# Sindhu-Hegde/jegal

Hardware: AMD Instinct MI355X
Metric: clips/sec (T=150 frames, 270x480) embedding extraction (higher is better)
Workload: dtype f16; 1 GPU; BASELINE configs[1]: synthetic batch=32 gesture-only (GestSync conv + JEGAL gesture encoder), uint8 150x270x480x3 clips resident in HBM, seeded synthetic weights; clips_per_gpu=32, frames=150, precision_mode=5, chunk=32, conv1_zero_tile_skip=True, dual_stream=True, parallelism=clip-sharded x1, no data-path collective

## Files before the change

### include/jegal_hip.h

```cpp
#ifndef JEGAL_HIP_H
#define JEGAL_HIP_H

#include <stdint.h>

#ifdef __cplusplus
extern "C" {
#endif

typedef struct jg_handle jg_handle;

enum { JG_OK = 0, JG_ERR_ARG = -1, JG_ERR_HIP = -2, JG_ERR_STATE = -3, JG_ERR_WEIGHT = -4 };

enum { JG_F32 = 0, JG_F16 = 1, JG_I64 = 2, JG_U8 = 3 };

enum {
    JG_PREC_FP16 = 0,
    JG_PREC_FP16_W2 = 1,
    JG_PREC_FP16_W2_ALL = 2,
    JG_PREC_FP16_BC = 3,
    JG_PREC_BF16 = 4,
    JG_PREC_FP16_RC = 5,
    JG_PREC_FP32 = 6
};

int jg_create(int device, jg_handle** out);
int jg_destroy(jg_handle* h);
const char* jg_last_error(jg_handle* h);
int jg_set_stream(jg_handle* h, void* hip_stream);
int jg_set_precision(jg_handle* h, int mode);
int jg_set_chunk(jg_handle* h, int clips_per_chunk);
int jg_set_option(jg_handle* h, const char* name, int value);
int jg_sync(jg_handle* h);

int jg_load_tensor(jg_handle* h, const char* name, const void* data_host, const int64_t* shape_host, int ndim, int dtype);
int jg_finalize_weights(jg_handle* h, int which);
int jg_clear_staged_tensors(jg_handle* h);

int jg_calibrate_gesture(jg_handle* h, const void* frames, int frames_dtype, int B, int T);

int jg_xlmr_encode(jg_handle* h, const int32_t* input_ids, const int32_t* attention_mask, int B, int L, float* out);
int jg_calibrate_xlmr(jg_handle* h, const int32_t* input_ids, const int32_t* attention_mask, int B, int L);

int jg_gestsync_clip(jg_handle* h, const void* frames, int frames_dtype, int B, int T, float* out_feats);
int jg_gestsync_clip_ragged(jg_handle* h, const void* frames, int frames_dtype, int B, int T, const int32_t* valid_frames_host, float* out_feats);
int jg_debug_conv1_pool(jg_handle* h, const void* frames_u8, int B, int T, int pad, void* out_f16);
typedef struct jg_gemm_check {
    const void* A; int64_t lda;
    const void* Wh; const void* Wl; int64_t ldw;
    int M, N, K;
    const float* scale; const float* bias;
    const float* bias_clip; int rpc, nclips;
    const float* res; int64_t ldr; int res_mod;
    int relu;
    float* out32; void* out16; int64_t ldc;
    const float* ln_w; const float* ln_b; const void* res16;
    int ln_mode; const float* ln_stats; const void* xres_hi; const void* xres_lo; void* out_lo; float* stat_out;
} jg_gemm_check;
int jg_debug_gemm_check(jg_handle* h, const jg_gemm_check* c);
typedef struct jg_conv_shape { int H, W, C, KH, KW, PH, PW, tap_table, rowmap, const_in; } jg_conv_shape;
int jg_debug_gemm_plan(const jg_gemm_check* c, const jg_conv_shape* conv, int a_tiled, int num_cu, int lanes_active, const char* const* opt_names,
                       const int* opt_values, int n_opts, char* name, int name_len, int* grid, int* lds, int* stagger);
int jg_debug_weight_form(int precision, int kind, int model, int keep32, int* form, int* lo_kept, int* uncalibrated);
int jg_debug_gemm_runs_lo(int form, int uncalibrated, int calibrating, int clip_bias, int* lo);
typedef struct jg_conv_check {
    const void* in;
    int nimg, H, W, C, KH, KW, SH, SW, PH, PW, reorder;
    const void* Wh; const void* Wl; int64_t ldw;
    int N, K;
    const float* scale; const float* bias;
    int relu;
    float* out32; void* out16; int64_t ldc;
    const int32_t* s2_host; int op; const void* const_in;
} jg_conv_check;
int jg_debug_conv_check(jg_handle* h, const jg_conv_check* c);
int jg_debug_maxpool(jg_handle* h, const void* in, int nimg, int H, int W, int C, const int32_t* s2_host, int in_op, const void* const_in, void* out);
int jg_debug_conv_rowmaps(jg_handle* h, const int32_t* s2_host, int NF, const int* OH, const int* OW, int nlayers, int32_t* const* map_host,
                          int32_t* const* base_host, int32_t* total_host);
int jg_debug_gemm32(jg_handle* h, const float* A, int64_t lda, const float* W, int64_t ldw, int M, int N, int K, const float* scale,
                    const float* bias, const float* res, int64_t ldr, int res_mod, int act, float* out, int64_t ldc);
int jg_debug_gemm_x3(jg_handle* h, const float* A, int64_t lda, const void* Wh, const void* Wl, int64_t ldw, int M, int N, int K,
                     const float* bias, const float* res, int64_t ldr, int res_mod, int relu, float* out, int64_t ldc);
int jg_debug_attention(jg_handle* h, const void* qkv, const float* keymask, int B, int S, int H, int dk, void* out);
int jg_debug_attention_gather(jg_handle* h, const void* qkv_pos, const void* pe_qkv, int Twin, int P, int shift, int B, int S, int H, void* out);
int jg_debug_attention32(jg_handle* h, const float* qkv, const float* keymask, int B, int S, int H, int dk, float* out);
int jg_debug_last_kernel(jg_handle* h, char* buf, int len);
int jg_debug_conv2_rowskip(jg_handle* h, int* rows);
int jg_debug_conv_rows(jg_handle* h, int64_t* computed, int64_t* full);
int jg_debug_gemm(jg_handle* h, int M, int N, int K, int mode, int iters, double* ms);
int jg_debug_gemm_ex(jg_handle* h, const void* a16, const void* w16, int M, int N, int K, int mode, int iters, double* ms);
int jg_gestsync_windows(jg_handle* h, const float* x, int N, float* out, float* out_conv);

int jg_mask_resize(jg_handle* h, const uint8_t* src, int T, int H, int W, const int32_t* mask_y, uint8_t* dst);

int jg_unpack_masked(jg_handle* h, const uint8_t* packed, int64_t packed_bytes, const int32_t* row0, const int64_t* offsets, int n_frames, uint8_t* dst);
int jg_mask_resize_packed(jg_handle* h, const uint8_t* packed, int64_t packed_bytes, const int64_t* offsets, int T, int H, int W,
                          const int32_t* mask_y, uint8_t* dst);

int jg_jegal_gestures(jg_handle* h, const float* feats, const float* mask, int B, int T, int align, float* out);
int jg_jegal_audio(jg_handle* h, const float* mel, int B, int Tm, float* out);
int jg_audio_len(int Tm);
int jg_jegal_audio_ragged(jg_handle* h, const float* mel, int B, int Tm, const int32_t* valid_tm_host, float* out);
int jg_logmel(jg_handle* h, const float* wav, int B, int n_samples, const float* mel_basis, float* out);
int jg_jegal_text(jg_handle* h, const float* states, const float* mask, int B, int L, float* out);
int jg_word_pool(jg_handle* h, const float* seq, int D, const int32_t* seg, int n_seg, float* dst, int dst_ld, int dst_col);
int jg_fuse_content(jg_handle* h, const float* fused, int rows, float* out);
int jg_l2norm(jg_handle* h, const float* in, float* out, int rows, int D);
int jg_extract_gesture(jg_handle* h, const void* frames, int frames_dtype, int B, int T, float* out_emb);

int jg_pool_mean(jg_handle* h, const float* x, const int32_t* offsets, int n, int D, float* out);
int jg_sim_rank(jg_handle* h, const float* e1, const float* e2, int n_local, int n_total, int row_offset, int D,
                int32_t* rank, int32_t* ties);
int jg_spot(jg_handle* h, const float* gesture, const float* content, const int32_t* g_offsets, const int32_t* c_offsets,
            const int32_t* target, int n_clips, int D, float temp, int32_t* pred, float* score);
int jg_asd(jg_handle* h, const float* query, const float* cand, const int32_t* c_offsets, int n, int D, float temp, int32_t* pred);

#define JG_COMM_ID_BYTES 128
int jg_comm_get_unique_id(char* id128_host);
int jg_comm_init(jg_handle* h, const char* id128_host, int rank, int world);
int jg_comm_destroy(jg_handle* h);
int jg_allgather(jg_handle* h, const void* send, void* recv, int64_t bytes_per_rank);
int jg_allreduce_sum_i64(jg_handle* h, int64_t* buf, int n);

enum { JG_ST_STACK = 0, JG_ST_CONV1, JG_ST_POOL, JG_ST_CONV, JG_ST_GEMM, JG_ST_ATTN, JG_ST_NORM, JG_ST_MISC, JG_ST_CONV1_AUX, JG_ST_COUNT };
int jg_profile_enable(jg_handle* h, int on);
int jg_profile_get(jg_handle* h, int stage, double* ms, int64_t* launches);
int jg_profile_reset(jg_handle* h);
const char* jg_stage_name(int stage);
int64_t jg_workspace_bytes(jg_handle* h);

#ifdef __cplusplus
}
#endif
#endif
```

### jegal_amd/_lib.py

```python
import ctypes
import os

import numpy as np
import torch

_HERE = os.path.dirname(os.path.abspath(__file__))
LIB_PATH = os.path.join(_HERE, "libjegal_hip.so")

JG_F32, JG_F16, JG_I64, JG_U8 = 0, 1, 2, 3
PREC_FP16, PREC_FP16_W2, PREC_FP16_W2_ALL, PREC_FP16_BC, PREC_BF16, PREC_FP16_RC, PREC_FP32 = 0, 1, 2, 3, 4, 5, 6
AUDIT_CONV, AUDIT_GESTSYNC, AUDIT_JEGAL, AUDIT_CONTENT, AUDIT_XLMR = 1, 2, 4, 8, 16
STAGES = ["stack_frames", "conv1", "maxpool", "conv2-fc6+audio_cnn", "gemm", "attention", "layernorm", "misc", "conv1_aux"]

_P = ctypes.c_void_p
_I = ctypes.c_int
_L = ctypes.c_int64
JG_ERR_ARG = -1


class GemmCheck(ctypes.Structure):
    _fields_ = [("A", _P), ("lda", _L), ("Wh", _P), ("Wl", _P), ("ldw", _L), ("M", _I), ("N", _I), ("K", _I),
                ("scale", _P), ("bias", _P), ("bias_clip", _P), ("rpc", _I), ("nclips", _I),
                ("res", _P), ("ldr", _L), ("res_mod", _I), ("relu", _I), ("out32", _P), ("out16", _P), ("ldc", _L),
                ("ln_w", _P), ("ln_b", _P), ("res16", _P),
                ("ln_mode", _I), ("ln_stats", _P), ("xres_hi", _P), ("xres_lo", _P), ("out_lo", _P), ("stat_out", _P)]
class ConvCheck(ctypes.Structure):
    _fields_ = [("in_", _P)] + [(k, _I) for k in ("nimg", "H", "W", "C", "KH", "KW", "SH", "SW", "PH", "PW", "reorder")] + [
        ("Wh", _P), ("Wl", _P), ("ldw", _L), ("N", _I), ("K", _I), ("scale", _P), ("bias", _P), ("relu", _I),
        ("out32", _P), ("out16", _P), ("ldc", _L), ("s2_host", ctypes.POINTER(ctypes.c_int32)), ("op", _I), ("const_in", _P)]
class ConvShape(ctypes.Structure):
    _fields_ = [(k, _I) for k in ("H", "W", "C", "KH", "KW", "PH", "PW", "tap_table", "rowmap", "const_in")]


_SIGS = {
    "jg_create": [_I, ctypes.POINTER(_P)],
    "jg_destroy": [_P],
    "jg_set_stream": [_P, _P],
    "jg_set_precision": [_P, _I],
    "jg_set_chunk": [_P, _I],
    "jg_set_option": [_P, ctypes.c_char_p, _I],
    "jg_sync": [_P],
    "jg_load_tensor": [_P, ctypes.c_char_p, _P, ctypes.POINTER(ctypes.c_int64), _I, _I],
    "jg_finalize_weights": [_P, _I],
    "jg_clear_staged_tensors": [_P],
    "jg_calibrate_gesture": [_P, _P, _I, _I, _I],
    "jg_gestsync_clip": [_P, _P, _I, _I, _I, _P],
    "jg_gestsync_clip_ragged": [_P, _P, _I, _I, _I, ctypes.POINTER(ctypes.c_int32), _P],
    "jg_gestsync_windows": [_P, _P, _I, _P, _P],
    "jg_debug_conv1_pool": [_P, _P, _I, _I, _I, _P],
    "jg_debug_gemm": [_P, _I, _I, _I, _I, _I, ctypes.POINTER(ctypes.c_double)],
    "jg_debug_gemm_ex": [_P, _P, _P, _I, _I, _I, _I, _I, ctypes.POINTER(ctypes.c_double)],
    "jg_debug_conv2_rowskip": [_P, ctypes.POINTER(ctypes.c_int)],
    "jg_debug_gemm_check": [_P, _P],
    "jg_debug_conv_check": [_P, _P],
    "jg_debug_maxpool": [_P, _P, _I, _I, _I, _I, ctypes.POINTER(ctypes.c_int32), _I, _P, _P],
    "jg_debug_conv_rowmaps": [_P, ctypes.POINTER(ctypes.c_int32), _I, ctypes.POINTER(_I), ctypes.POINTER(_I), _I, ctypes.POINTER(_P), ctypes.POINTER(_P),
                              ctypes.POINTER(ctypes.c_int32)],
    "jg_debug_gemm_plan": [_P, _P, _I, _I, _I, ctypes.POINTER(ctypes.c_char_p), ctypes.POINTER(_I), _I, ctypes.c_char_p, _I,
                           ctypes.POINTER(_I), ctypes.POINTER(_I), ctypes.POINTER(_I)],
    "jg_debug_weight_form": [_I, _I, _I, _I, ctypes.POINTER(_I), ctypes.POINTER(_I), ctypes.POINTER(_I)],
    "jg_debug_gemm_runs_lo": [_I, _I, _I, _I, ctypes.POINTER(_I)],
    "jg_debug_gemm32": [_P, _P, _L, _P, _L, _I, _I, _I, _P, _P, _P, _L, _I, _I, _P, _L],
    "jg_debug_gemm_x3": [_P, _P, _L, _P, _P, _L, _I, _I, _I, _P, _P, _L, _I, _I, _P, _L],
    "jg_debug_attention": [_P, _P, _P, _I, _I, _I, _I, _P],
    "jg_debug_attention_gather": [_P, _P, _P, _I, _I, _I, _I, _I, _I, _P],
    "jg_debug_attention32": [_P, _P, _P, _I, _I, _I, _I, _P],
    "jg_debug_last_kernel": [_P, ctypes.c_char_p, _I],
    "jg_debug_conv_rows": [_P, ctypes.POINTER(ctypes.c_int64), ctypes.POINTER(ctypes.c_int64)],
    "jg_jegal_gestures": [_P, _P, _P, _I, _I, _I, _P],
    "jg_jegal_audio": [_P, _P, _I, _I, _P],
    "jg_jegal_audio_ragged": [_P, _P, _I, _I, ctypes.POINTER(ctypes.c_int32), _P],
    "jg_audio_len": [_I],
    "jg_logmel": [_P, _P, _I, _I, _P, _P],
    "jg_mask_resize": [_P, _P, _I, _I, _I, _P, _P],
    "jg_unpack_masked": [_P, _P, ctypes.c_int64, _P, _P, _I, _P],
    "jg_mask_resize_packed": [_P, _P, ctypes.c_int64, _P, _I, _I, _I, _P, _P],
    "jg_jegal_text": [_P, _P, _P, _I, _I, _P],
    "jg_xlmr_encode": [_P, _P, _P, _I, _I, _P],
    "jg_calibrate_xlmr": [_P, _P, _P, _I, _I],
    "jg_word_pool": [_P, _P, _I, _P, _I, _P, _I, _I],
    "jg_fuse_content": [_P, _P, _I, _P],
    "jg_l2norm": [_P, _P, _P, _I, _I],
    "jg_extract_gesture": [_P, _P, _I, _I, _I, _P],
    "jg_pool_mean": [_P, _P, _P, _I, _I, _P],
    "jg_sim_rank": [_P, _P, _P, _I, _I, _I, _I, _P, _P],
    "jg_spot": [_P, _P, _P, _P, _P, _P, _I, _I, ctypes.c_float, _P, _P],
    "jg_asd": [_P, _P, _P, _P, _I, _I, ctypes.c_float, _P],
    "jg_comm_get_unique_id": [ctypes.c_char_p],
    "jg_comm_init": [_P, ctypes.c_char_p, _I, _I],
    "jg_comm_destroy": [_P],
    "jg_allgather": [_P, _P, _P, ctypes.c_int64],
    "jg_allreduce_sum_i64": [_P, _P, _I],
    "jg_profile_enable": [_P, _I],
    "jg_profile_get": [_P, _I, ctypes.POINTER(ctypes.c_double), ctypes.POINTER(ctypes.c_int64)],
    "jg_profile_reset": [_P],
}
EXPORTS = sorted(list(_SIGS) + ["jg_last_error", "jg_stage_name", "jg_workspace_bytes"])

_lib = None


def load_library():
    global _lib
    if _lib is not None:
        return _lib
    if not os.path.exists(LIB_PATH):
        raise RuntimeError(
            f"{LIB_PATH} not found: build it with `python -c 'import __graft_entry__ as g; g.build()'` "
            "(or `make -C jegal_amd/csrc`).  jegal_amd has no CPU/PyTorch fallback.")
    lib = ctypes.CDLL(LIB_PATH)
    for name, args in _SIGS.items():
        fn = getattr(lib, name)
        fn.argtypes = args
        fn.restype = _I
    lib.jg_last_error.argtypes = [_P]
    lib.jg_last_error.restype = ctypes.c_char_p
    lib.jg_stage_name.argtypes = [_I]
    lib.jg_stage_name.restype = ctypes.c_char_p
    lib.jg_workspace_bytes.argtypes = [_P]
    lib.jg_workspace_bytes.restype = ctypes.c_int64
    _lib = lib
    return lib


def gemm_plan(num_cu=256, lanes_active=False, opts=None, conv=None, a_tiled=False, **fields):
    lib = load_library()
    c = GemmCheck()
    ptr_fields = {k for k, t in GemmCheck._fields_ if t is _P}
    for k, v in fields.items():
        if k in ptr_fields:
            v = 1 if isinstance(v, torch.Tensor) or bool(v) else None
        setattr(c, k, v)
    opts = dict(opts or {})
    num_cu = opts.pop("num_cu", num_cu)
    names = (ctypes.c_char_p * max(len(opts), 1))(*[k.encode() for k in opts])
    values = (_I * max(len(opts), 1))(*[int(v) for v in opts.values()])
    cs = ConvShape(**{k: int(v) for k, v in conv.items()}) if conv is not None else None
    name = ctypes.create_string_buffer(128)
    grid, lds, stagger = _I(), _I(), _I()
    rc = lib.jg_debug_gemm_plan(ctypes.byref(c), ctypes.byref(cs) if cs is not None else None, int(bool(a_tiled)), int(num_cu), int(bool(lanes_active)),
                                names, values, len(opts), name, 128, ctypes.byref(grid), ctypes.byref(lds), ctypes.byref(stagger))
    if rc != 0:
        raise JegalError(f"jg_debug_gemm_plan: bad arguments or unknown option ({rc})", rc)
    return name.value.decode(), grid.value, lds.value, stagger.value


WEIGHT_FORMS = ["single", "split", "bias_corrected", "runtime_corrected"]


def weight_form(precision, kind, model, keep32=False):
    form, lo, unc = _I(), _I(), _I()
    rc = load_library().jg_debug_weight_form(int(precision), int(kind), int(model), int(bool(keep32)), ctypes.byref(form), ctypes.byref(lo), ctypes.byref(unc))
    if rc != 0:
        raise JegalError(f"jg_debug_weight_form: bad arguments ({rc})", rc)
    return WEIGHT_FORMS[form.value], bool(lo.value), bool(unc.value)


def gemm_runs_lo(form, uncalibrated=False, calibrating=False, clip_bias=False):
    lo = _I()
    rc = load_library().jg_debug_gemm_runs_lo(WEIGHT_FORMS.index(form), int(bool(uncalibrated)), int(bool(calibrating)), int(bool(clip_bias)), ctypes.byref(lo))
    if rc != 0:
        raise JegalError(f"jg_debug_gemm_runs_lo: bad arguments ({rc})", rc)
    return bool(lo.value)


class JegalError(RuntimeError):
    def __init__(self, msg, code=None):
        super().__init__(msg)
        self.code = code


def _ptr(t):
    return None if t is None else ctypes.c_void_p(t.data_ptr())


class Engine:

    _cache = {}

    @classmethod
    def get(cls, device=None):
        if not torch.cuda.is_available():
            raise RuntimeError("jegal_amd needs a HIP device (torch.cuda.is_available() is False); there is no CPU fallback")
        dev = torch.device("cuda", torch.cuda.current_device()) if device is None else torch.device(device)
        idx = dev.index if dev.index is not None else torch.cuda.current_device()
        if idx not in cls._cache:
            cls._cache[idx] = cls(idx)
        return cls._cache[idx]

    def __init__(self, device_index=0, precision=None):
        self.lib = load_library()
        self.device = torch.device("cuda", device_index)
        torch.cuda.init()
        with torch.cuda.device(self.device):
            torch.zeros(1, device=self.device)
        h = _P()
        rc = self.lib.jg_create(device_index, ctypes.byref(h))
        if rc != 0:
            raise JegalError(f"jg_create({device_index}) failed with {rc}")
        self.h = h
        self.precision = PREC_FP16_RC
        if precision is not None:
            self.set_precision(precision)
        self.finalized = 0

    def close(self):
        if getattr(self, "h", None):
            self.lib.jg_destroy(self.h)
            self.h = None
            for k, v in list(Engine._cache.items()):
                if v is self:
                    del Engine._cache[k]

    def _ck(self, rc):
        if rc != 0:
            raise JegalError(f"libjegal_hip error {rc}: {self.lib.jg_last_error(self.h).decode()}", rc)

    def _bind_stream(self):
        self._ck(self.lib.jg_set_stream(self.h, _P(torch.cuda.current_stream(self.device).cuda_stream)))

    def set_precision(self, mode):
        self._ck(self.lib.jg_set_precision(self.h, mode))
        self.precision = int(mode)

    def set_option(self, name, value):
        self._ck(self.lib.jg_set_option(self.h, name.encode(), int(value)))

    def set_chunk(self, clips):
        self._ck(self.lib.jg_set_chunk(self.h, int(clips)))

    def load_tensors(self, state_dict):
        for name, val in state_dict.items():
            if isinstance(val, torch.Tensor):
                val = val.detach().cpu().numpy()
            arr = np.asarray(val)
            if arr.dtype == np.float16:
                code = JG_F16
            elif arr.dtype == np.int64:
                code = JG_I64
            else:
                arr = arr.astype(np.float32, copy=False)
                code = JG_F32
            arr = np.ascontiguousarray(arr)
            shape = (ctypes.c_int64 * max(arr.ndim, 1))(*arr.shape)
            self._ck(self.lib.jg_load_tensor(self.h, name.encode(), arr.ctypes.data_as(_P), shape, arr.ndim, code))

    def finalize(self, which, clear_staged=True):
        with torch.cuda.device(self.device):
            self._ck(self.lib.jg_finalize_weights(self.h, which))
        if clear_staged:
            self._ck(self.lib.jg_clear_staged_tensors(self.h))
        self.finalized |= which

    def _f32(self, t):
        return torch.as_tensor(t, device=self.device).to(torch.float32).contiguous()

    def _i32(self, a):
        if isinstance(a, torch.Tensor):
            return a.to(device=self.device, dtype=torch.int32).contiguous()
        return torch.as_tensor(np.ascontiguousarray(np.asarray(a, np.int32)), device=self.device)

    def sync(self):
        self._ck(self.lib.jg_sync(self.h))

    def calibrate(self, frames=None):
        self._bind_stream()
        if frames is None:
            self._ck(self.lib.jg_calibrate_gesture(self.h, None, JG_U8, 0, 0))
            return
        frames, code, B, T = self._frames_arg(frames)
        self._ck(self.lib.jg_calibrate_gesture(self.h, _ptr(frames), code, B, T))

    def _frames_arg(self, frames):
        if not isinstance(frames, torch.Tensor):
            frames = torch.as_tensor(frames)
        if frames.dim() != 5 or tuple(frames.shape[2:]) != (270, 480, 3):
            raise ValueError(f"frames must be (B,T,270,480,3), got {tuple(frames.shape)}")
        if frames.shape[0] == 0 or frames.shape[1] == 0:
            raise ValueError("frames must hold at least one clip of at least one frame")
        frames = frames.to(self.device)
        if frames.dtype == torch.uint8:
            code = JG_U8
        elif frames.dtype.is_floating_point:
            frames, code = frames.to(torch.float32), JG_F32
        else:
            raise ValueError(f"frames must be uint8 or floating point, got {frames.dtype}")
        return frames.contiguous(), code, frames.shape[0], frames.shape[1]

    def _out_arg(self, out, shape):
        if out is None:
            return torch.empty(shape, dtype=torch.float32, device=self.device)
        if (not isinstance(out, torch.Tensor) or out.device != self.device or out.dtype != torch.float32
                or tuple(out.shape) != tuple(shape) or not out.is_contiguous()):
            raise ValueError(f"out must be a contiguous float32 tensor of shape {tuple(shape)} on {self.device}")
        return out

    def gestsync_clip(self, frames, lengths=None):
        self._bind_stream()
        frames, code, B, T = self._frames_arg(frames)
        out = torch.empty((B, T, 1024), dtype=torch.float32, device=self.device)
        if lengths is None:
            self._ck(self.lib.jg_gestsync_clip(self.h, _ptr(frames), code, B, T, _ptr(out)))
            return out
        v = [int(x) for x in lengths]
        if len(v) != B:
            raise ValueError("lengths needs one entry per clip")
        self._ck(self.lib.jg_gestsync_clip_ragged(self.h, _ptr(frames), code, B, T, (ctypes.c_int32 * B)(*v), _ptr(out)))
        return out

    def debug_gemm(self, M, N, K, mode=0, iters=10, a16=None, w16=None):
        self._bind_stream()
        ms = ctypes.c_double()
        for t, shp in ((a16, (M, K)), (w16, (N, K))):
            if t is not None and (t.dtype != torch.float16 or tuple(t.shape) != shp or not t.is_contiguous() or t.device != self.device):
                raise ValueError(f"debug_gemm operand must be a contiguous fp16 {shp} tensor on {self.device}")
        self._ck(self.lib.jg_debug_gemm_ex(self.h, _ptr(a16), _ptr(w16), M, N, K, mode, iters, ctypes.byref(ms)))
        return ms.value

    def debug_gemm_check(self, **kw):
        self._bind_stream()
        c = GemmCheck()
        for k, v in kw.items():
            if isinstance(v, torch.Tensor):
                if v.device != self.device:
                    raise ValueError(f"debug_gemm_check: {k} must be on {self.device}")
                v = v.data_ptr()
            setattr(c, k, v)
        self._ck(self.lib.jg_debug_gemm_check(self.h, ctypes.byref(c)))

    def debug_conv_check(self, **kw):
        self._bind_stream()
        c = ConvCheck()
        s2 = kw.pop("s2_host", None)
        for k, v in kw.items():
            if isinstance(v, torch.Tensor):
                if v.device != self.device:
                    raise ValueError(f"debug_conv_check: {k} must be on {self.device}")
                v = v.data_ptr()
            setattr(c, "in_" if k == "in" else k, v)
        if s2 is not None:
            s2 = [int(x) for x in s2]
            if len(s2) != c.nimg:
                raise ValueError("debug_conv_check: s2_host needs one entry per image")
            keep = (ctypes.c_int32 * len(s2))(*s2)
            c.s2_host = ctypes.cast(keep, ctypes.POINTER(ctypes.c_int32))
        self._ck(self.lib.jg_debug_conv_check(self.h, ctypes.byref(c)))

    def debug_maxpool(self, x, out, s2_host=None, in_op=0, const_in=None):
        self._bind_stream()
        nimg, H, W, C = x.shape
        s2 = None
        if s2_host is not None:
            s2 = [int(v) for v in s2_host]
            if len(s2) != nimg:
                raise ValueError("debug_maxpool: s2_host needs one entry per image")
            s2 = (ctypes.c_int32 * nimg)(*s2)
        self._ck(self.lib.jg_debug_maxpool(self.h, _ptr(x), nimg, H, W, C, s2, int(in_op), _ptr(const_in), _ptr(out)))

    def debug_conv_rowmaps(self, s2_host, layers, fill=-1):
        self._bind_stream()
        s2 = np.ascontiguousarray(np.asarray(s2_host, np.int32))
        NF, nl = int(s2.size), len(layers)
        maps = [np.full(NF * oh * ow, fill, np.int32) for oh, ow in layers]
        bases = [np.full(NF + 1, fill, np.int32) for _ in layers]
        totals = np.full(max(nl, 1), fill, np.int32)
        i32p = ctypes.POINTER(ctypes.c_int32)
        OH = (_I * max(nl, 1))(*[oh for oh, _ in layers])
        OW = (_I * max(nl, 1))(*[ow for _, ow in layers])
        mp = (_P * max(nl, 1))(*[m.ctypes.data for m in maps])
        bp = (_P * max(nl, 1))(*[b.ctypes.data for b in bases])
        self._ck(self.lib.jg_debug_conv_rowmaps(self.h, s2.ctypes.data_as(i32p), NF, OH, OW, nl, mp, bp, totals.ctypes.data_as(i32p)))
        return [(maps[l], bases[l], int(totals[l])) for l in range(nl)]

    def debug_gemm32(self, A, lda, W, ldw, M, N, K, out, ldc, scale=None, bias=None, res=None, ldr=0, res_mod=0, act=0):
        self._bind_stream()
        self._ck(self.lib.jg_debug_gemm32(self.h, _ptr(A), lda, _ptr(W), ldw, M, N, K, _ptr(scale), _ptr(bias), _ptr(res), ldr, res_mod, act,
                                          _ptr(out), ldc))

    def debug_gemm_x3(self, A, lda, Wh, Wl, ldw, M, N, K, out, ldc, bias=None, res=None, ldr=0, res_mod=0, relu=0):
        self._bind_stream()
        self._ck(self.lib.jg_debug_gemm_x3(self.h, _ptr(A), lda, _ptr(Wh), _ptr(Wl), ldw, M, N, K, _ptr(bias), _ptr(res), ldr, res_mod, relu,
                                           _ptr(out), ldc))

    def debug_attention(self, qkv, keymask, B, S, H, dk, out):
        self._bind_stream()
        self._ck(self.lib.jg_debug_attention(self.h, _ptr(qkv), _ptr(keymask), B, S, H, dk, _ptr(out)))

    def debug_attention_gather(self, qkv_pos, pe_qkv, Twin, P, shift, B, S, H, out):
        self._bind_stream()
        self._ck(self.lib.jg_debug_attention_gather(self.h, _ptr(qkv_pos), _ptr(pe_qkv), Twin, P, shift, B, S, H, _ptr(out)))

    def debug_attention32(self, qkv, keymask, B, S, H, dk, out):
        self._bind_stream()
        self._ck(self.lib.jg_debug_attention32(self.h, _ptr(qkv), _ptr(keymask), B, S, H, dk, _ptr(out)))

    def debug_last_kernel(self):
        buf = ctypes.create_string_buffer(128)
        self._ck(self.lib.jg_debug_last_kernel(self.h, buf, 128))
        return buf.value.decode()

    def debug_conv2_rowskip(self):
        rows = ctypes.c_int()
        self._ck(self.lib.jg_debug_conv2_rowskip(self.h, ctypes.byref(rows)))
        return rows.value

    def debug_conv_rows(self):
        c, f = (ctypes.c_int64 * 4)(), (ctypes.c_int64 * 4)()
        self._ck(self.lib.jg_debug_conv_rows(self.h, c, f))
        return list(c), list(f)

    def debug_conv1_pool(self, frames_u8, pad):
        self._bind_stream()
        frames_u8 = frames_u8.to(self.device).contiguous()
        B, T = frames_u8.shape[:2]
        out = torch.empty((B * (T + 2 * pad - 4), 43, 78, 64), dtype=torch.float16, device=self.device)
        self._ck(self.lib.jg_debug_conv1_pool(self.h, _ptr(frames_u8), B, T, pad, _ptr(out)))
        return out

    def gestsync_windows(self, x, return_feats=False):
        self._bind_stream()
        x = self._f32(x)
        if tuple(x.shape[1:]) != (3, 25, 270, 480):
            raise ValueError(f"x must be (N,3,25,270,480), got {tuple(x.shape)}")
        N = x.shape[0]
        out = torch.empty((N, 1024, 21), dtype=torch.float32, device=self.device)
        oc = torch.empty((N, 512, 21), dtype=torch.float32, device=self.device) if return_feats else None
        self._ck(self.lib.jg_gestsync_windows(self.h, _ptr(x), N, _ptr(out), _ptr(oc)))
        return (out, oc) if return_feats else out

    def extract_gesture(self, frames, out=None):
        self._bind_stream()
        frames, code, B, T = self._frames_arg(frames)
        if T > 500:
            raise ValueError("clips are limited to 500 frames (JEGAL's positional table, modules.py:136)")
        out = self._out_arg(out, (B, T, 512))
        self._ck(self.lib.jg_extract_gesture(self.h, _ptr(frames), code, B, T, _ptr(out)))
        return out

    def jegal_gestures(self, feats, mask=None, align=False):
        self._bind_stream()
        feats = self._f32(feats)
        B, T, D = feats.shape
        if D != 1024:
            raise ValueError("visual feats must have 1024 channels")
        m = None if mask is None else self._f32(mask).reshape(B, T)
        out = torch.empty((B, T, 512), dtype=torch.float32, device=self.device)
        self._ck(self.lib.jg_jegal_gestures(self.h, _ptr(feats), _ptr(m), B, T, int(bool(align)), _ptr(out)))
        return out

    def audio_len(self, Tm):
        return int(self.lib.jg_audio_len(int(Tm)))

    def jegal_audio(self, mel, valid_len=None):
        self._bind_stream()
        mel = self._f32(mel)
        B, Tm, F = mel.shape
        if F != 80:
            raise ValueError("mel must have 80 bands")
        out = torch.empty((B, self.audio_len(Tm), 256), dtype=torch.float32, device=self.device)
        if valid_len is None:
            self._ck(self.lib.jg_jegal_audio(self.h, _ptr(mel), B, Tm, _ptr(out)))
            return out
        v = [int(x) for x in valid_len]
        if len(v) != B:
            raise ValueError("valid_len needs one entry per clip")
        self._ck(self.lib.jg_jegal_audio_ragged(self.h, _ptr(mel), B, Tm, (ctypes.c_int32 * B)(*v), _ptr(out)))
        return out

    def mask_resize(self, frames_u8, mask_y):
        self._bind_stream()
        frames_u8 = frames_u8.to(self.device).contiguous()
        if frames_u8.dtype != torch.uint8 or frames_u8.dim() != 4 or frames_u8.shape[-1] != 3:
            raise ValueError("frames must be uint8 (T,H,W,3)")
        T, H, W, _ = frames_u8.shape
        my = torch.as_tensor(mask_y, dtype=torch.int32).to(self.device).contiguous()
        if my.numel() != T:
            raise ValueError("mask_y needs one entry per frame")
        out = torch.empty((T, 270, 480, 3), dtype=torch.uint8, device=self.device)
        self._ck(self.lib.jg_mask_resize(self.h, _ptr(frames_u8), T, H, W, _ptr(my), _ptr(out)))
        return out

    def unpack_masked(self, packed, row0, offsets, dst):
        self._bind_stream()
        F = row0.numel()
        if (packed.dtype != torch.uint8 or row0.dtype != torch.int32 or offsets.dtype != torch.int64 or dst.dtype != torch.uint8
                or offsets.numel() != F or dst.numel() != F * 270 * 480 * 3 or not dst.is_contiguous() or not packed.is_contiguous()):
            raise ValueError("unpack_masked: packed uint8, row0 int32 (F), offsets int64 (F), dst uint8 (F,270,480,3)")
        self._ck(self.lib.jg_unpack_masked(self.h, _ptr(packed), packed.numel(), _ptr(row0), _ptr(offsets), F, _ptr(dst)))
        return dst

    def mask_resize_packed(self, packed, offsets, mask_y, H, W, dst):
        self._bind_stream()
        F = mask_y.numel()
        if (packed.dtype != torch.uint8 or mask_y.dtype != torch.int32 or offsets.dtype != torch.int64 or dst.dtype != torch.uint8
                or offsets.numel() != F or dst.numel() != F * 270 * 480 * 3 or not dst.is_contiguous() or not packed.is_contiguous()):
            raise ValueError("mask_resize_packed: packed uint8, offsets int64 (F), mask_y int32 (F), dst uint8 (F,270,480,3)")
        self._ck(self.lib.jg_mask_resize_packed(self.h, _ptr(packed), packed.numel(), _ptr(offsets), F, int(H), int(W), _ptr(mask_y), _ptr(dst)))
        return dst

    def logmel(self, wav, mel_basis):
        self._bind_stream()
        wav = self._f32(wav)
        mb = self._f32(mel_basis)
        B, n = wav.shape
        out = torch.empty((B, n // 160, 80), dtype=torch.float32, device=self.device)
        self._ck(self.lib.jg_logmel(self.h, _ptr(wav), B, n, _ptr(mb), _ptr(out)))
        return out

    def jegal_text(self, states, mask=None):
        self._bind_stream()
        states = self._f32(states)
        B, L, D = states.shape
        if D != 768:
            raise ValueError("text states must have 768 channels")
        m = None if mask is None else self._f32(mask).reshape(B, L)
        out = torch.empty((B, L, 256), dtype=torch.float32, device=self.device)
        self._ck(self.lib.jg_jegal_text(self.h, _ptr(states), _ptr(m), B, L, _ptr(out)))
        return out

    def xlmr_encode(self, input_ids, attention_mask=None):
        self._bind_stream()
        ids = self._i32(input_ids)
        if ids.ndim != 2:
            raise ValueError("input_ids must be (B, L)")
        B, L = ids.shape
        m = None
        if attention_mask is not None:
            m = self._i32(attention_mask)
            if tuple(m.shape) != (B, L):
                raise ValueError("attention_mask must have the shape of input_ids")
        out = torch.empty((B, L, 768), dtype=torch.float32, device=self.device)
        self._ck(self.lib.jg_xlmr_encode(self.h, _ptr(ids), _ptr(m), B, L, _ptr(out)))
        return out

    def calibrate_xlmr(self, input_ids=None, attention_mask=None):
        self._bind_stream()
        if input_ids is None:
            self._ck(self.lib.jg_calibrate_xlmr(self.h, None, None, 0, 0))
            return
        ids = self._i32(input_ids)
        if ids.ndim != 2:
            raise ValueError("input_ids must be (B, L)")
        m = None if attention_mask is None else self._i32(attention_mask)
        if m is not None and tuple(m.shape) != tuple(ids.shape):
            raise ValueError("attention_mask must have the shape of input_ids")
        self._ck(self.lib.jg_calibrate_xlmr(self.h, _ptr(ids), _ptr(m), ids.shape[0], ids.shape[1]))

    def word_pool(self, seq, segments, dst, dst_col):
        self._bind_stream()
        seg = self._i32(segments).reshape(-1, 3)
        if seg.shape[0] == 0:
            return
        self._ck(self.lib.jg_word_pool(self.h, _ptr(seq), seq.shape[-1], _ptr(seg), seg.shape[0], _ptr(dst), dst.shape[-1], dst_col))

    def fuse_content(self, fused):
        self._bind_stream()
        fused = self._f32(fused)
        rows = fused.numel() // 512
        out = torch.empty_like(fused)
        self._ck(self.lib.jg_fuse_content(self.h, _ptr(fused), rows, _ptr(out)))
        return out

    def l2norm(self, x):
        self._bind_stream()
        x = self._f32(x)
        out = torch.empty_like(x)
        D = x.shape[-1]
        self._ck(self.lib.jg_l2norm(self.h, _ptr(x), _ptr(out), x.numel() // D, D))
        return out

    def pool_mean(self, x, offsets):
        self._bind_stream()
        x = self._f32(x)
        off = self._i32(offsets)
        n = off.numel() - 1
        out = torch.empty((n, x.shape[-1]), dtype=torch.float32, device=self.device)
        self._ck(self.lib.jg_pool_mean(self.h, _ptr(x), _ptr(off), n, x.shape[-1], _ptr(out)))
        return out

    def sim_rank(self, e1, e2, row_offset=0):
        self._bind_stream()
        e1, e2 = self._f32(e1), self._f32(e2)
        n_local, D = e1.shape
        rank = torch.empty(n_local, dtype=torch.int32, device=self.device)
        ties = torch.empty(n_local, dtype=torch.int32, device=self.device)
        self._ck(self.lib.jg_sim_rank(self.h, _ptr(e1), _ptr(e2), n_local, e2.shape[0], row_offset, D, _ptr(rank), _ptr(ties)))
        return rank, ties

    def spot(self, gesture, content, g_offsets, c_offsets, targets, temp=0.07):
        self._bind_stream()
        g, c = self._f32(gesture), self._f32(content)
        goh, coh, tgh = (np.asarray(a, np.int64) for a in (g_offsets, c_offsets, targets))
        n = tgh.size
        if goh.size != n + 1 or coh.size != n + 1:
            raise ValueError("g_offsets / c_offsets need one entry more than targets")
        T, W = np.diff(goh), np.diff(coh)
        if n and (T.min() <= 0 or T.max() > 8192 or W.min() <= 0 or W.max() > 1024 or (tgh < 0).any() or (tgh >= W).any()):
            raise ValueError("jg_spot limits: 1..8192 frames and 1..1024 words per clip, 0 <= target < words")
        go, co, tg = self._i32(g_offsets), self._i32(c_offsets), self._i32(targets)
        pred = torch.empty(n, dtype=torch.int32, device=self.device)
        score = torch.empty(n, dtype=torch.float32, device=self.device)
        self._ck(self.lib.jg_spot(self.h, _ptr(g), _ptr(c), _ptr(go), _ptr(co), _ptr(tg), n, g.shape[-1], temp, _ptr(pred), _ptr(score)))
        return pred, score

    def asd(self, query, cand, c_offsets, temp=0.07):
        self._bind_stream()
        q, c = self._f32(query), self._f32(cand)
        co = self._i32(c_offsets)
        n = q.shape[0]
        pred = torch.empty((n, 3), dtype=torch.int32, device=self.device)
        self._ck(self.lib.jg_asd(self.h, _ptr(q), _ptr(c), _ptr(co), n, q.shape[-1], temp, _ptr(pred)))
        return pred

    @staticmethod
    def comm_unique_id():
        buf = ctypes.create_string_buffer(128)
        rc = load_library().jg_comm_get_unique_id(buf)
        if rc != 0:
            raise JegalError(f"jg_comm_get_unique_id failed with {rc} (librccl.so not loadable?)")
        return buf.raw

    def comm_init(self, unique_id, rank, world):
        with torch.cuda.device(self.device):
            self._ck(self.lib.jg_comm_init(self.h, bytes(unique_id), int(rank), int(world)))
        self.comm_world = int(world)

    def comm_destroy(self):
        self._ck(self.lib.jg_comm_destroy(self.h))
        self.comm_world = 1

    def allgather(self, x):
        self._bind_stream()
        x = x.to(self.device).contiguous()
        out = torch.empty((getattr(self, "comm_world", 1) * x.shape[0],) + tuple(x.shape[1:]), dtype=x.dtype, device=self.device)
        self._ck(self.lib.jg_allgather(self.h, _ptr(x), _ptr(out), x.numel() * x.element_size()))
        return out

    def allreduce_sum_i64(self, counts):
        self._bind_stream()
        t = torch.as_tensor(counts, dtype=torch.int64).to(self.device).contiguous().clone()
        self._ck(self.lib.jg_allreduce_sum_i64(self.h, _ptr(t), t.numel()))
        return t

    def profile(self, on, only=None):
        self._ck(self.lib.jg_profile_enable(self.h, 2 + STAGES.index(only) if (on and only) else int(bool(on))))

    def profile_reset(self):
        self._ck(self.lib.jg_profile_reset(self.h))

    def profile_get(self):
        res = {}
        for i, name in enumerate(STAGES):
            ms, n = ctypes.c_double(), ctypes.c_int64()
            self._ck(self.lib.jg_profile_get(self.h, i, ctypes.byref(ms), ctypes.byref(n)))
            res[name] = (ms.value, n.value)
        return res

    def workspace_bytes(self):
        return int(self.lib.jg_workspace_bytes(self.h))
```

### jegal_amd/csrc/checks.hip

```cpp
#include "engine.h"

using namespace engine;

namespace {
int check_result(jg_handle* h, hipError_t e, const char* what) {
    if (e == hipErrorInvalidValue) JG_FAIL(h, JG_ERR_ARG, "%s: the launcher rejects this shape / argument set", what);
    if (e != hipSuccess) JG_FAIL(h, JG_ERR_HIP, "%s: %s", what, hipGetErrorString(e));
    return JG_OK;
}
GemmArgs gemm_check_args(const jg_gemm_check* c) {
    GemmArgs a;
    std::memset(&a, 0, sizeof(a));
    a.A = static_cast<const f16*>(c->A); a.lda = c->lda;
    a.Wh = static_cast<const f16*>(c->Wh); a.Wl = static_cast<const f16*>(c->Wl); a.ldw = c->ldw;
    a.M = c->M; a.N = c->N; a.K = c->K;
    a.scale = c->scale; a.bias = c->bias;
    a.bias_clip = c->bias_clip; a.rpc = c->rpc; a.nclips = c->nclips;
    a.res = c->res; a.ldr = c->ldr; a.res_mod = c->res_mod; a.relu = c->relu;
    a.out32 = c->out32; a.out16 = static_cast<f16*>(c->out16); a.ldc = c->ldc;
    a.ln_w = c->ln_w; a.ln_b = c->ln_b; a.ln_flavour = LN_STD;
    a.res16 = static_cast<const f16*>(c->res16);
    a.ln_mode = c->ln_mode; a.ln_stats = c->ln_stats;
    a.xres_hi = static_cast<const f16*>(c->xres_hi); a.xres_lo = static_cast<const f16*>(c->xres_lo);
    a.out_lo = static_cast<f16*>(c->out_lo); a.stat_out = c->stat_out;
    return a;
}
}

extern "C" {

int jg_debug_conv2_rowskip(jg_handle* h, int* rows) {
    ENTER(h);
    if (!rows) JG_FAIL(h, JG_ERR_ARG, "rows is NULL");
    *rows = 0;
    if (!h->last_rowskip) return JG_OK;
    HIPCHK(h, hipStreamSynchronize(h->stream));
    HIPCHK(h, hipMemcpy(rows, h->last_rowskip, sizeof(int), hipMemcpyDeviceToHost));
    return JG_OK;
}

int jg_debug_conv_rows(jg_handle* h, int64_t* computed, int64_t* full) {
    ENTER(h);
    if (!computed || !full) JG_FAIL(h, JG_ERR_ARG, "null buffer");
    for (int l = 0; l < 4; ++l) computed[l] = full[l] = 0;
    if (!h->last_conv_totals) return JG_OK;
    HIPCHK(h, hipStreamSynchronize(h->stream));
    int t[4];
    HIPCHK(h, hipMemcpy(t, h->last_conv_totals, sizeof(t), hipMemcpyDeviceToHost));
    for (int l = 0; l < 4; ++l) { computed[l] = t[l]; full[l] = h->last_conv_full[l]; }
    return JG_OK;
}

int jg_debug_conv1_pool(jg_handle* h, const void* frames_u8, int B, int T, int pad, void* out_f16) {
    ENTER(h);
    if (!h->gs.m.ready) JG_FAIL(h, JG_ERR_STATE, "GestSync weights not finalized");
    if (!frames_u8 || !out_f16 || B <= 0 || pad < 0 || pad > 12 || T + 2 * pad < 5)
        JG_FAIL(h, JG_ERR_ARG, "bad arguments (need 0 <= pad <= 12 and T + 2*pad >= 5)");
    h->ws.reset();
    const long sw = 3, sh = (long)FW * 3, st = (long)FH * FW * 3, sb = (long)T * st;
    unsigned* zscr;
    return gs_conv1_stage(h, frames_u8, 1, sb, st, sh, sw, 1, B, T, pad, static_cast<f16*>(out_f16), true, &zscr);
}

int jg_debug_gemm(jg_handle* h, int M, int N, int K, int mode, int iters, double* ms) {
    return jg_debug_gemm_ex(h, nullptr, nullptr, M, N, K, mode, iters, ms);
}

int jg_debug_gemm_ex(jg_handle* h, const void* a16, const void* w16, int M, int N, int K, int mode, int iters, double* ms) {
    if (!h || !ms || M <= 0 || N <= 0 || K <= 0 || iters <= 0) return JG_ERR_ARG;
    ENTER(h);
    h->ws.reset();
    f16 *A, *Wh, *Wl, *o16;
    float *bias, *x32;
    RET(wsalloc(h, (size_t)M * K, &A));
    RET(wsalloc(h, (size_t)N * K, &Wh));
    RET(wsalloc(h, (size_t)N * K, &Wl));
    RET(wsalloc(h, pad128(M) * N, &o16));
    RET(wsalloc(h, pad128(M) * N, &x32));
    RET(wsalloc(h, (size_t)N, &bias));
    if (a16) HIPCHK(h, hipMemcpyAsync(A, a16, (size_t)M * K * 2, hipMemcpyDeviceToDevice, h->stream));
    else HIPCHK(h, hipMemsetAsync(A, 0x3c, (size_t)M * K * 2, h->stream));
    if (w16) HIPCHK(h, hipMemcpyAsync(Wh, w16, (size_t)N * K * 2, hipMemcpyDeviceToDevice, h->stream));
    else HIPCHK(h, hipMemsetAsync(Wh, 0x2c, (size_t)N * K * 2, h->stream));
    HIPCHK(h, hipMemsetAsync(Wl, 0x1c, (size_t)N * K * 2, h->stream));
    HIPCHK(h, hipMemsetAsync(bias, 0, (size_t)N * 4, h->stream));
    HIPCHK(h, hipMemsetAsync(x32, 0, (size_t)M * N * 4, h->stream));
    GemmArgs a;
    std::memset(&a, 0, sizeof(a));
    a.A = A; a.lda = K; a.Wh = Wh; a.Wl = (mode & 1) ? Wl : nullptr; a.ldw = K;
    a.M = M; a.N = N; a.K = K; a.bias = bias; a.ldc = N; a.relu = (mode >> 2) & 1;
    if (mode & 2) { a.res = x32; a.ldr = N; a.out32 = x32; } else { a.out16 = o16; }
    if (mode & 8) {
        a.res = nullptr; a.out32 = nullptr;
        a.res16 = o16; a.out16 = o16;
        a.ln_w = bias; a.ln_b = bias; a.ln_flavour = LN_STD;
    }
    if (mode & 48) {
        float* stats;
        RET(wsalloc(h, (size_t)pad128(M) * 2, &stats));
        HIPCHK(h, hipMemsetAsync(stats, 0, (size_t)M * 2 * 4, h->stream));
        a.res = nullptr; a.out32 = nullptr; a.scale = bias; a.ln_stats = stats;
        if (mode & 16) { a.ln_mode = 1; a.out16 = o16; }
        else {
            f16* lo;
            float* part;
            RET(wsalloc(h, pad128(M) * N, &lo));
            RET(wsalloc(h, (size_t)pad128(M) * (N / 64) * 2, &part));
            a.ln_mode = 2; a.relu = 0; a.xres_hi = o16; a.xres_lo = lo; a.out16 = o16; a.out_lo = lo; a.stat_out = part;
        }
    }
    hipEvent_t e0, e1;
    HIPCHK(h, hipEventCreate(&e0));
    HIPCHK(h, hipEventCreate(&e1));
    HIPCHK(h, LAUNCH(h, launch_gemm, a, false, h->opts, h->stream));
    HIPCHK(h, hipEventRecord(e0, h->stream));
    for (int i = 0; i < iters; ++i) HIPCHK(h, LAUNCH(h, launch_gemm, a, false, h->opts, h->stream));
    HIPCHK(h, hipEventRecord(e1, h->stream));
    HIPCHK(h, hipEventSynchronize(e1));
    float t = 0.f;
    HIPCHK(h, hipEventElapsedTime(&t, e0, e1));
    (void)hipEventDestroy(e0);
    (void)hipEventDestroy(e1);
    *ms = t / iters;
    return JG_OK;
}

int jg_debug_gemm_check(jg_handle* h, const jg_gemm_check* c) {
    ENTER(h);
    h->kname[0] = 0;
    if (!c || !c->A || !c->Wh || c->M <= 0 || c->N <= 0 || c->K <= 0 || c->lda < c->K || c->ldw < c->K || (!c->out32 && !c->out16) ||
        ((c->out32 || (c->out16 && !c->ln_w)) && c->ldc < c->N) || (c->res && (c->ldr < c->N || c->res_mod < 0)) ||
        (c->bias_clip && (c->rpc <= 0 || c->nclips <= 0)) || c->relu < 0 || c->relu > 2 || c->ln_mode < 0 || c->ln_mode > 2)
        JG_FAIL(h, JG_ERR_ARG, "jg_debug_gemm_check: bad arguments");
    const GemmArgs a = gemm_check_args(c);
    EngineOpts o = h->opts;
    o.kname = h->kname;
    return check_result(h, LAUNCH(h, launch_gemm, a, false, o, h->stream), "launch_gemm");
}

int jg_debug_conv_check(jg_handle* h, const jg_conv_check* c) {
    ENTER(h);
    h->kname[0] = 0;
    if (!c || !c->in || !c->Wh || c->nimg <= 0 || c->H <= 0 || c->W <= 0 || c->C < 8 || (c->C & (c->C - 1)) || c->KH <= 0 || c->KW <= 0 || c->KH > 15 ||
        c->KW > 15 || c->SH <= 0 || c->SW <= 0 || c->PH < 0 || c->PW < 0 || c->H + 2 * c->PH < c->KH || c->W + 2 * c->PW < c->KW || c->N <= 0 ||
        (long)c->KH * c->KW * c->C != c->K || c->ldw < c->K || (!c->out32 && !c->out16) || c->ldc < c->N || c->relu < 0 || c->relu > 1 || c->op < 0 ||
        c->op > 3 || (c->const_in && (!c->s2_host || c->op == 0)))
        JG_FAIL(h, JG_ERR_ARG, "jg_debug_conv_check: bad arguments (K = KH KW C, C a power of two >= 8, relu 0 / 1, op 0..3, const_in needs s2_host and op >= 1)");
    ConvGeom g = geom(c->H, c->W, c->C, c->KH, c->KW, c->SH, c->SW, c->PH, c->PW, c->reorder != 0);
    const long M = (long)c->nimg * g.OH * g.OW;
    if (M >= (1L << 31)) JG_FAIL(h, JG_ERR_ARG, "jg_debug_conv_check: too many output pixels");
    if (c->s2_host) {
        for (int i = 0; i < c->nimg; ++i)
            if (c->s2_host[i] < 0 || c->s2_host[i] > 255 || conv_skip_decode(c->s2_host[i], c->op) >= g.OH)
                JG_FAIL(h, JG_ERR_ARG, "jg_debug_conv_check: s2[%d] = %d outside 0..255 or leaves image %d no output row", i, c->s2_host[i], i);
    }
    GemmArgs a;
    std::memset(&a, 0, sizeof(a));
    a.A = static_cast<const f16*>(c->in);
    a.Wh = static_cast<const f16*>(c->Wh); a.Wl = static_cast<const f16*>(c->Wl); a.ldw = c->ldw;
    a.M = (int)M; a.N = c->N; a.K = c->K;
    a.scale = c->scale; a.bias = c->bias; a.relu = c->relu;
    a.out32 = c->out32; a.out16 = static_cast<f16*>(c->out16); a.ldc = c->ldc;
    EngineOpts o = h->opts;
    o.kname = h->kname;
    if (c->s2_host) {
        GemmShape q = gemm_shape(a, false);
        q.set_geom(g);
        q.rowmap = true; q.const_in = c->const_in != nullptr;
        if (!plan_gemm(q, o).ok()) JG_FAIL(h, JG_ERR_ARG, "launch_gemm: the launcher rejects this shape / argument set");
        h->ws.reset();
        int32_t* s2;
        int* totals;
        ConvRowMap rm;
        rm.OH = g.OH; rm.OW = g.OW; rm.op = c->op;
        RET(wsalloc(h, (size_t)c->nimg, &s2));
        RET(wsalloc(h, (size_t)M, &rm.map));
        RET(wsalloc(h, (size_t)c->nimg + 1, &rm.base));
        RET(wsalloc(h, (size_t)64, &totals));
        rm.total = totals;
        RET(upload_i32_async(h, c->s2_host, (size_t)c->nimg, s2));
        const int rc = check_result(h, launch_conv_rowmaps(s2, c->nimg, &rm, 1, h->stream), "launch_conv_rowmaps");
        if (rc != JG_OK) return rc;
        g.rowmap = rm.map; g.rows_total = rm.total;
        g.in_op = c->op - 1; g.const_in = static_cast<const f16*>(c->const_in);
    }
    a.g = g;
    return check_result(h, LAUNCH(h, launch_gemm, a, true, o, h->stream), "launch_gemm");
}

int jg_debug_maxpool(jg_handle* h, const void* in, int nimg, int H, int W, int C, const int32_t* s2_host, int in_op, const void* const_in, void* out) {
    ENTER(h);
    h->kname[0] = 0;
    if (!in || !out || nimg <= 0 || H < 3 || W < 3 || C <= 0 || C % 8 || (s2_host != nullptr) != (const_in != nullptr) || in_op < 0 || in_op > 3)
        JG_FAIL(h, JG_ERR_ARG, "jg_debug_maxpool: bad arguments (C %% 8 == 0, H, W >= 3, s2_host and const_in together, in_op 0..3)");
    int32_t* s2 = nullptr;
    if (s2_host) {
        for (int i = 0; i < nimg; ++i)
            if (s2_host[i] < 0 || s2_host[i] > 255 || conv_skip_decode(s2_host[i], in_op) > H)
                JG_FAIL(h, JG_ERR_ARG, "jg_debug_maxpool: s2[%d] = %d outside 0..255 or past the image's %d rows", i, s2_host[i], H);
        h->ws.reset();
        RET(wsalloc(h, (size_t)nimg, &s2));
        RET(upload_i32_async(h, s2_host, (size_t)nimg, s2));
    }
    const int rc = check_result(h, LAUNCH(h, launch_maxpool3x3s2, static_cast<const f16*>(in), static_cast<f16*>(out), nimg, H, W, C, h->stream,
                                          static_cast<const int*>(s2), in_op, static_cast<const f16*>(const_in)), "launch_maxpool3x3s2");
    if (rc == JG_OK) record_kernel(h->kname, "%s", "maxpool_kernel");
    return rc;
}

int jg_debug_conv_rowmaps(jg_handle* h, const int32_t* s2_host, int NF, const int* OH, const int* OW, int nlayers, int32_t* const* map_host,
                          int32_t* const* base_host, int32_t* total_host) {
    ENTER(h);
    h->kname[0] = 0;
    if (!s2_host || !OH || !OW || !map_host || !base_host || !total_host || NF <= 0) JG_FAIL(h, JG_ERR_ARG, "jg_debug_conv_rowmaps: bad arguments");
    if (nlayers < 1 || nlayers > 4) JG_FAIL(h, JG_ERR_ARG, "launch_conv_rowmaps: the launcher rejects this shape / argument set");
    for (int l = 0; l < nlayers; ++l) {
        if (OH[l] <= 0 || OW[l] <= 0 || !map_host[l] || !base_host[l]) JG_FAIL(h, JG_ERR_ARG, "jg_debug_conv_rowmaps: bad layer %d", l);
        for (int i = 0; i < NF; ++i)
            if (s2_host[i] < 0 || s2_host[i] > 255 || conv_skip_decode(s2_host[i], l) > OH[l])
                JG_FAIL(h, JG_ERR_ARG, "jg_debug_conv_rowmaps: s2[%d] = %d outside 0..255 or past layer %d's %d rows", i, s2_host[i], l, OH[l]);
    }
    h->ws.reset();
    int32_t* s2;
    int* totals;
    ConvRowMap rm[4];
    RET(wsalloc(h, (size_t)NF, &s2));
    RET(wsalloc(h, (size_t)64, &totals));
    RET(upload_i32_async(h, s2_host, (size_t)NF, s2));
    for (int l = 0; l < nlayers; ++l) {
        const size_t n = (size_t)NF * OH[l] * OW[l];
        rm[l].OH = OH[l]; rm[l].OW = OW[l]; rm[l].op = l;
        RET(wsalloc(h, n, &rm[l].map));
        RET(wsalloc(h, (size_t)NF + 1, &rm[l].base));
        rm[l].total = totals + l;
        HIPCHK(h, hipMemcpy(rm[l].map, map_host[l], n * sizeof(int), hipMemcpyHostToDevice));
    }
    const int rc = check_result(h, launch_conv_rowmaps(s2, NF, rm, nlayers, h->stream), "launch_conv_rowmaps");
    if (rc != JG_OK) return rc;
    record_kernel(h->kname, "%s", "conv_rowmap_scan_kernel+conv_rowmap_fill_kernel");
    HIPCHK(h, hipStreamSynchronize(h->stream));
    for (int l = 0; l < nlayers; ++l) {
        HIPCHK(h, hipMemcpy(map_host[l], rm[l].map, (size_t)NF * OH[l] * OW[l] * sizeof(int), hipMemcpyDeviceToHost));
        HIPCHK(h, hipMemcpy(base_host[l], rm[l].base, ((size_t)NF + 1) * sizeof(int), hipMemcpyDeviceToHost));
        HIPCHK(h, hipMemcpy(total_host + l, rm[l].total, sizeof(int), hipMemcpyDeviceToHost));
    }
    return JG_OK;
}

int jg_debug_gemm_plan(const jg_gemm_check* c, const jg_conv_shape* conv, int a_tiled, int num_cu, int lanes_active, const char* const* opt_names,
                       const int* opt_values, int n_opts, char* name, int name_len, int* grid, int* lds, int* stagger) {
    if (!c || c->M <= 0 || c->N <= 0 || c->K <= 0 || num_cu <= 0 || n_opts < 0 || (n_opts && (!opt_names || !opt_values)) || !name || name_len <= 0 ||
        !grid || !lds || !stagger)
        return JG_ERR_ARG;
    GemmShape s = gemm_shape(gemm_check_args(c), false);
    s.a_tiled = a_tiled != 0;
    if (conv) {
        s.conv = true;
        s.H = conv->H; s.W = conv->W; s.C = conv->C; s.KH = conv->KH; s.KW = conv->KW; s.PH = conv->PH; s.PW = conv->PW;
        s.tap_table = conv->tap_table; s.rowmap = conv->rowmap != 0; s.const_in = conv->const_in != 0;
    }
    EngineOpts o;
    o.num_cu = num_cu;
    o.lanes_active = lanes_active != 0;
    for (int i = 0; i < n_opts; ++i)
        if (!opt_names[i] || !engine_opts_set(o, opt_names[i], opt_values[i])) return JG_ERR_ARG;
    const GemmPlan p = plan_gemm(s, o);
    snprintf(name, (size_t)name_len, "%s", p.name);
    *grid = (int)p.grid; *lds = (int)p.lds; *stagger = p.stagger;
    return JG_OK;
}

int jg_debug_weight_form(int precision, int kind, int model, int keep32, int* form, int* lo_kept_out, int* uncalibrated) {
    if (precision < JG_PREC_FP16 || precision > JG_PREC_FP32 || kind < LK_CONV || kind > LK_XLMR || model < 1 || model > 3 || !form || !lo_kept_out ||
        !uncalibrated)
        return JG_ERR_ARG;
    const WeightForm f = weight_form(precision, kind, model);
    *form = f; *lo_kept_out = lo_kept(f, keep32 != 0); *uncalibrated = starts_uncalibrated(f, kind);
    return JG_OK;
}

int jg_debug_gemm_runs_lo(int form, int uncalibrated, int calibrating, int clip_bias, int* lo) {
    if (form < WF_SINGLE || form > WF_RUNTIME_CORRECTED || !lo) return JG_ERR_ARG;
    *lo = runs_with_lo((WeightForm)form, uncalibrated != 0, calibrating != 0, clip_bias != 0);
    return JG_OK;
}

int jg_debug_gemm32(jg_handle* h, const float* A, int64_t lda, const float* W, int64_t ldw, int M, int N, int K, const float* scale,
                    const float* bias, const float* res, int64_t ldr, int res_mod, int act, float* out, int64_t ldc) {
    ENTER(h);
    h->kname[0] = 0;
    if (!A || !W || !out || M <= 0 || N <= 0 || K <= 0 || lda < K || ldw < K || ldc < N || (res && (ldr < N || res_mod < 0)) || act < 0 || act > 2)
        JG_FAIL(h, JG_ERR_ARG, "jg_debug_gemm32: bad arguments");
    Gemm32Args a;
    std::memset(&a, 0, sizeof(a));
    a.A = A; a.lda = lda; a.W = W; a.ldw = ldw; a.M = M; a.N = N; a.K = K;
    a.scale = scale; a.bias = bias; a.res = res; a.ldr = ldr; a.res_mod = res_mod; a.out = out; a.ldc = ldc; a.act = act;
    return check_result(h, launch_gemm32(a, h->stream, h->kname), "launch_gemm32");
}

int jg_debug_gemm_x3(jg_handle* h, const float* A, int64_t lda, const void* Wh, const void* Wl, int64_t ldw, int M, int N, int K,
                     const float* bias, const float* res, int64_t ldr, int res_mod, int relu, float* out, int64_t ldc) {
    ENTER(h);
    h->kname[0] = 0;
    if (!A || !Wh || !Wl || !out || M <= 0 || N <= 0 || K <= 0 || lda < K || ldw < K || ldc < N || (res && (ldr < N || res_mod < 0)) ||
        relu < 0 || relu > 1)
        JG_FAIL(h, JG_ERR_ARG, "jg_debug_gemm_x3: bad arguments");
    GemmX3Args a;
    std::memset(&a, 0, sizeof(a));
    a.A = A; a.lda = lda; a.Wh = static_cast<const f16*>(Wh); a.Wl = static_cast<const f16*>(Wl); a.ldw = ldw; a.M = M; a.N = N; a.K = K;
    a.bias = bias; a.res = res; a.ldr = ldr; a.res_mod = res_mod; a.out = out; a.ldc = ldc; a.relu = relu;
    return check_result(h, launch_gemm_x3(a, h->stream, h->kname), "launch_gemm_x3");
}

int jg_debug_attention(jg_handle* h, const void* qkv, const float* keymask, int B, int S, int H, int dk, void* out) {
    ENTER(h);
    h->kname[0] = 0;
    if (!qkv || !out || B <= 0 || S <= 0 || H <= 0 || (dk != 64 && dk != 96)) JG_FAIL(h, JG_ERR_ARG, "jg_debug_attention: bad arguments");
    EngineOpts o = h->opts;
    o.kname = h->kname;
    return check_result(h, LAUNCH(h, launch_attention, static_cast<const f16*>(qkv), keymask, B, S, H, dk, static_cast<f16*>(out), o, h->stream),
                        "launch_attention");
}

int jg_debug_attention_gather(jg_handle* h, const void* qkv_pos, const void* pe_qkv, int Twin, int P, int shift, int B, int S, int H, void* out) {
    ENTER(h);
    h->kname[0] = 0;
    if (!qkv_pos || !pe_qkv || !out || B <= 0 || S <= 0 || H <= 0 || Twin <= 0 || P <= 0 || B % Twin)
        JG_FAIL(h, JG_ERR_ARG, "jg_debug_attention_gather: bad arguments (B must be a multiple of Twin)");
    if (h->bf16) JG_FAIL(h, JG_ERR_STATE, "jg_debug_attention_gather: the gather form is an fp16-build kernel (the clip path's layer 0)");
    const AttnGather g{static_cast<const f16*>(pe_qkv), Twin, P, shift};
    return check_result(h, launch_attention_gather(static_cast<const f16*>(qkv_pos), g, B, S, H, static_cast<f16*>(out), h->stream, h->kname),
                        "launch_attention_gather");
}

int jg_debug_attention32(jg_handle* h, const float* qkv, const float* keymask, int B, int S, int H, int dk, float* out) {
    ENTER(h);
    h->kname[0] = 0;
    if (!qkv || !out || B <= 0 || S <= 0 || H <= 0) JG_FAIL(h, JG_ERR_ARG, "jg_debug_attention32: bad arguments");
    return check_result(h, launch_attention32(qkv, keymask, B, S, H, dk, out, h->stream, h->kname), "launch_attention32");
}

int jg_debug_last_kernel(jg_handle* h, char* buf, int len) {
    if (!h || !buf || len <= 0) return JG_ERR_ARG;
    snprintf(buf, (size_t)len, "%s", h->kname);
    return JG_OK;
}

}
```

### jegal_amd/csrc/conv1.hip

```cpp
#include "common.h"

#ifdef JG_CLOCK_STAMPS
__device__ unsigned long long jg_clock_stamps_conv1[2 * 1024];
extern "C" int jg_clock_read_conv1(unsigned long long* out, int n) {
    return hipMemcpyFromSymbol(out, HIP_SYMBOL(jg_clock_stamps_conv1), sizeof(unsigned long long) * (n < 2048 ? n : 2048)) == hipSuccess ? 0 : 1;
}
#endif
#include <cstdio>
#include <cstdlib>
#include <cstring>

struct Conv1Args {
    const uint8_t* src;
    int nclip, T, pad, P;
    const f16* Wd;
    float scale;
    f16* out;
    f16* edge;
    f16* dump;
    int nstrips;
    float invP;
    int zskip;
    const unsigned* zmask;
    const f16* zconst;
    int fill_partial;
};

namespace {
constexpr int IH = 270, IW = 480;
constexpr int PH = 43, PW = 78;
constexpr int TROWS = 16;
constexpr int ROW_PITCH = 3744;
constexpr int TILE_BYTES = TROWS * ROW_PITCH;
__device__ __host__ constexpr int slot_off(int x) { return 32 * x + 16 * (x / 3); }
constexpr int ROW_TILES = 22, COL_TILES = 5;
constexpr int CONV_BYTES = 4 * 8 * 32 * 16;
constexpr int CARRY_BYTES = 8 * 32 * 16;
constexpr int OFF_CONV = 2 * TILE_BYTES;
constexpr int OFF_CARRY = OFF_CONV + 2 * CONV_BYTES;
constexpr int OFF_INIT = OFF_CARRY + 2 * CARRY_BYTES;
constexpr int OFF_LIVE = OFF_INIT + 32;
constexpr int OFF_SKIP = OFF_INIT + 256;
constexpr int MAX_WG_STRIPS = 640;
constexpr int LDS_BYTES = OFF_SKIP + 4 * MAX_WG_STRIPS;
constexpr int MAX_WGS = 1024;
constexpr int DUMP_HALVES_PER_WG = 256 * 8;
}

typedef uint32_t u32x3 __attribute__((ext_vector_type(3)));
struct C1Regs { u32x3 w[2][5]; };

__device__ __forceinline__ f16x8 max8(f16x8 a, f16x8 b) {
    return __builtin_elementwise_max(a, b);
}

__device__ __forceinline__ int conv1_s2_of_mask(unsigned sk) {
    const int L = __builtin_ctz(~sk);
    constexpr int C2_OH = (PH - 5) / 2 + 1;
    const int rs = L >= 2 ? L - 2 : 0;
    return rs < C2_OH ? rs : C2_OH - 1;
}

struct Strips {
    int s_lo, r_hi, GX;
    const unsigned* tab;
    bool use_skip;
    __device__ __forceinline__ bool any() const { return s_lo < r_hi && GX > 0; }
    __device__ __forceinline__ unsigned zero_bands(int k) const {
        return use_skip ? (unsigned)__builtin_amdgcn_readfirstlane((int)tab[k]) : 0u;
    }
};
__device__ __forceinline__ Strips conv1_strips(const Conv1Args& a, const char* smem) {
    const int G32 = (int)gridDim.x;
    const int xcd = blockIdx.x & 7, xidx = blockIdx.x >> 3;
    const int GX = (G32 + 7 - xcd) >> 3;
    const int per = (a.nstrips + 7) >> 3;
    const int r_lo = xcd * per, r_hi = (r_lo + per < a.nstrips) ? r_lo + per : a.nstrips;
    return Strips{r_lo + xidx, r_hi, GX, reinterpret_cast<const unsigned*>(smem + OFF_SKIP), a.zmask != nullptr};
}
__device__ __forceinline__ void strip_split(int strip, int& nf, int& j) {
    nf = (int)((unsigned)strip / 5u);
    j = strip - nf * 5;
}
__device__ __forceinline__ unsigned skip_of(unsigned z) { return z & ((z << 1) | 1u); }
struct Walk {
    int strip, rt;
    int k;
    unsigned skip;
    unsigned z;
    bool done;
};
template <class F>
__device__ __forceinline__ void walk_next(const Strips& S, Walk& q, F&& on_strip) {
    if (q.done) return;
    while (true) {
        if (++q.rt == ROW_TILES) {
            q.rt = 0;
            q.strip += S.GX;
            ++q.k;
            if (q.strip >= S.r_hi) { q.done = true; return; }
            q.z = S.zero_bands(q.k);
            q.skip = skip_of(q.z);
            on_strip(q.strip, q.skip);
        }
        if (!((q.skip >> q.rt) & 1u)) return;
    }
}
template <class F>
__device__ __forceinline__ Walk walk_first(const Strips& S, F&& on_strip) {
    Walk q = {S.s_lo, -1, 0, 0u, 0u, !S.any()};
    if (q.done) return q;
    q.z = S.zero_bands(0);
    q.skip = skip_of(q.z);
    on_strip(q.strip, q.skip);
    walk_next(S, q, on_strip);
    return q;
}

__device__ __forceinline__ bool tile_live(const char* smem, int t) {
    return __builtin_amdgcn_readfirstlane(*reinterpret_cast<const int*>(smem + OFF_LIVE + (t & 1) * 4)) != 0;
}
__device__ __forceinline__ bool tile_is_zero(const char* smem, int t) {
    const int4 fl = *reinterpret_cast<const int4*>(smem + OFF_INIT + (t & 1) * 16);
    return __builtin_amdgcn_readfirstlane(fl.x | fl.y | fl.z | fl.w) == 0;
}

struct Mfma32 {
    static constexpr int NSTEP = 49, NCB = 1;
    static constexpr int DEPTH = 6;
    typedef f32x16 Acc;
    const int chalf, r, h;
    f16x8 wreg[49];
    const char* base;
    __device__ __forceinline__ Mfma32(const f16* Wd, int lane, int chalf_) : chalf(chalf_), r(lane & 31), h(lane >> 5) {
#pragma unroll
        for (int s = 0; s < 49; ++s)
            wreg[s] = *reinterpret_cast<const f16x8*>(Wd + ((long)(s * 64 + chalf * 32 + r) * 16 + 8 * h));
    }
    __device__ __forceinline__ void set_tile(const char* cur) { base = cur + 112 * r + 16 * h; }
    __device__ __forceinline__ f16x8 frag(int gi) const {
        const int q = gi / 49, s = gi - q * 49;
        const int kh = s / 7, kw = s - kh * 7;
        return *reinterpret_cast<const f16x8*>(base + (6 * q + kh) * ROW_PITCH + 32 * kw + 16 * (kw / 3));
    }
    __device__ __forceinline__ static void zero(Acc& acc) {
#pragma unroll
        for (int x = 0; x < 16; ++x) acc[x] = 0.f;
    }
    __device__ __forceinline__ void step(Acc& acc, int s, int, f16x8 f) const {
        acc = __builtin_amdgcn_mfma_f32_32x32x16_f16(wreg[s], f, acc, 0, 0, 0);
    }
    __device__ __forceinline__ void store(const Acc& acc, char* cbuf, int mb, float scale) const {
#pragma unroll
        for (int g = 0; g < 4; ++g) {
            const f16x4 hv = {(f16)fmaxf(acc[4 * g] * scale, 0.f), (f16)fmaxf(acc[4 * g + 1] * scale, 0.f),
                              (f16)fmaxf(acc[4 * g + 2] * scale, 0.f), (f16)fmaxf(acc[4 * g + 3] * scale, 0.f)};
            *reinterpret_cast<f16x4*>(cbuf + ((mb * 8 + chalf * 4 + g) * 32 + r) * 16 + 8 * h) = hv;
        }
    }
};
struct Mfma16 {
    static constexpr int NSTEP = 25, NCB = 2;
    static constexpr int DEPTH = 4;
    struct Acc { f32x4 v[2][2]; };
    const int chalf, n16, kq, sel, half, colp;
    f16x8 wreg[25][2];
    int lb_row, lb_32, lb_224;
    int st_off;
    const char *p_row, *p_32, *p_224;
    __device__ __forceinline__ static void step_slots(int t, int& kha, int& kwa, int& khb, int& kwb) {
        if (t < 21) { kha = 2 * (t / 7); kwa = t % 7; khb = kha + 1; kwb = kwa; }
        else if (t == 21) { kha = khb = 6; kwa = 1; kwb = 2; }
        else if (t == 22) { kha = khb = 6; kwa = 4; kwb = 5; }
        else if (t == 23) { kha = khb = 6; kwa = 0; kwb = 6; }
        else { kha = khb = 6; kwa = 3; kwb = 4; }
    }
    __device__ __forceinline__ Mfma16(const f16* Wd, int lane, int chalf_)
        : chalf(chalf_), n16(lane & 15), kq(lane >> 4), sel(kq & 1), half(kq >> 1),
          colp((n16 >= 4 && n16 < 12) ? 2 * (n16 - 4) : (n16 < 4 ? 2 * n16 + 1 : 2 * (n16 - 8) + 1)) {
#pragma unroll
        for (int t = 0; t < 25; ++t) {
            int kha, kwa, khb, kwb;
            step_slots(t, kha, kwa, khb, kwb);
            const int sl = sel ? khb * 7 + kwb : kha * 7 + kwa;
#pragma unroll
            for (int ob = 0; ob < 2; ++ob) {
                wreg[t][ob] = *reinterpret_cast<const f16x8*>(Wd + ((long)(sl * 64 + chalf * 32 + ob * 16 + n16) * 16 + 8 * half));
                if (t == 24 && sel) wreg[t][ob] = f16x8{0, 0, 0, 0, 0, 0, 0, 0};
            }
        }
        const int lb = 112 * colp + 16 * half;
        lb_row = lb + sel * ROW_PITCH; lb_32 = lb + sel * 32; lb_224 = lb + sel * 224;
        st_off = ((chalf * 4 + (kq >> 1)) * 32 + colp) * 16 + 8 * (kq & 1);
    }
    __device__ __forceinline__ void set_tile(const char* cur) {
        p_row = cur + lb_row;
        p_32 = cur + lb_32;
        p_224 = cur + lb_224;
    }
    __device__ __forceinline__ f16x8 frag(int gi) const {
        const int q = gi / 50, st = (gi - q * 50) >> 1, cb = gi & 1;
        int kha, kwa, khb, kwb;
        step_slots(st, kha, kwa, khb, kwb);
        const int off = (6 * q + kha) * ROW_PITCH + 32 * kwa + 16 * (kwa / 3) + 1792 * cb;
        const char* pb = st < 21 ? p_row : (st == 23 ? p_224 : p_32);
        return *reinterpret_cast<const f16x8*>(pb + off);
    }
    __device__ __forceinline__ static void zero(Acc& acc) {
#pragma unroll
        for (int ob = 0; ob < 2; ++ob)
#pragma unroll
            for (int cb = 0; cb < 2; ++cb) acc.v[ob][cb] = f32x4{0.f, 0.f, 0.f, 0.f};
    }
    __device__ __forceinline__ void step(Acc& acc, int st, int cb, f16x8 f) const {
        acc.v[0][cb] = __builtin_amdgcn_mfma_f32_16x16x32_f16(wreg[st][0], f, acc.v[0][cb], 0, 0, 0);
        acc.v[1][cb] = __builtin_amdgcn_mfma_f32_16x16x32_f16(wreg[st][1], f, acc.v[1][cb], 0, 0, 0);
    }
    __device__ __forceinline__ void store(const Acc& acc, char* cbuf, int mb, float scale) const {
#pragma unroll
        for (int ob = 0; ob < 2; ++ob)
#pragma unroll
            for (int cb = 0; cb < 2; ++cb) {
                const f32x4 v = acc.v[ob][cb];
                const f16x4 hv = {(f16)fmaxf(v.x * scale, 0.f), (f16)fmaxf(v.y * scale, 0.f), (f16)fmaxf(v.z * scale, 0.f), (f16)fmaxf(v.w * scale, 0.f)};
                *reinterpret_cast<f16x4*>(cbuf + st_off + ((mb * 8 + ob * 2) * 32 + cb * 16) * 16) = hv;
            }
    }
};

template <class Form>
__device__ __forceinline__ void conv1_mfma_role(const f16* Wd, float scale, char* smem, int lane, int wave) {
    constexpr int NSTEP = Form::NSTEP, NCB = Form::NCB, DEPTH = Form::DEPTH, NFRAG = 2 * NSTEP * NCB;
    const int mb0 = (wave >> 1) & 1;
    Form F(Wd, lane, wave & 1);
#ifdef JG_CLOCK_STAMPS
    const unsigned long long ck0 = __builtin_amdgcn_s_memtime(), rt0 = __builtin_amdgcn_s_memrealtime();
#endif
    for (int t = 0;; ++t) {
        __syncthreads();
        if (!tile_live(smem, t)) break;
        F.set_tile(smem + (t & 1) * TILE_BYTES + 3 * mb0 * ROW_PITCH);
        char* cbuf = smem + OFF_CONV + (t & 1) * CONV_BYTES;
        if (tile_is_zero(smem, t)) {
#pragma unroll
            for (int q = 0; q < 2; ++q) {
                typename Form::Acc acc;
                Form::zero(acc);
#pragma unroll
                for (int st = 0; st < 2; ++st)
#pragma unroll
                    for (int cb = 0; cb < NCB; ++cb) F.step(acc, st, cb, F.frag((q * NSTEP + st) * NCB + cb));
                F.store(acc, cbuf, mb0 + 2 * q, scale);
            }
            continue;
        }
        f16x8 fr[DEPTH];
#pragma unroll
        for (int gi = 0; gi < DEPTH; ++gi) fr[gi] = F.frag(gi);
#pragma unroll
        for (int q = 0; q < 2; ++q) {
            typename Form::Acc acc;
            Form::zero(acc);
#pragma unroll
            for (int st = 0; st < NSTEP; ++st)
#pragma unroll
                for (int cb = 0; cb < NCB; ++cb) {
                    const int gi = (q * NSTEP + st) * NCB + cb;
                    F.step(acc, st, cb, fr[gi % DEPTH]);
                    if (gi + DEPTH < NFRAG) fr[gi % DEPTH] = F.frag(gi + DEPTH);
                    __builtin_amdgcn_sched_barrier(0);
                }
            F.store(acc, cbuf, mb0 + 2 * q, scale);
        }
    }
#ifdef JG_CLOCK_STAMPS
    if (wave == 0 && lane == 0 && blockIdx.x < 1024) {
        jg_clock_stamps_conv1[2 * blockIdx.x] = __builtin_amdgcn_s_memtime() - ck0;
        jg_clock_stamps_conv1[2 * blockIdx.x + 1] = __builtin_amdgcn_s_memrealtime() - rt0;
    }
#endif
}

template <bool M16>
__global__ __launch_bounds__(512, 2) void conv1_direct_kernel(Conv1Args a) {
    extern __shared__ __attribute__((aligned(16))) char smem[];
    const int tid = threadIdx.x, lane = tid & 63;
    const int wave = __builtin_amdgcn_readfirstlane(tid >> 6);
    const Strips S = conv1_strips(a, smem);
    if (!S.any()) return;
    if (S.use_skip) {
        unsigned* tab = reinterpret_cast<unsigned*>(smem + OFF_SKIP);
        for (int k = tid; k < MAX_WG_STRIPS; k += 512) {
            const int strip = S.s_lo + k * S.GX;
            int nf, j;
            strip_split(strip, nf, j);
            tab[k] = strip < S.r_hi ? a.zmask[nf] : 0u;
        }
        __syncthreads();
    }
    if (wave >= 4) {
        const int ltid = tid - 256;
        const int row0 = ltid / 25, g0 = ltid - row0 * 25;
        const int it1 = ltid + 256;
        const bool has1 = it1 < TROWS * 25;
        const int row1 = has1 ? it1 / 25 : 0, g1 = has1 ? it1 - row1 * 25 : 0;

        uint32_t fb0_lo = (uint32_t)(uintptr_t)a.src, fb0_hi = (uint32_t)((uintptr_t)a.src >> 32);
        uint32_t fdelta[5] = {0, 0, 0, 0, 0};
        uint32_t ioff[2] = {0, 0};
        auto decode = [&](int strip, int& nf, int& j, int& b, int& pp) {
            strip_split(strip, nf, j);
            b = (int)((float)nf * a.invP);
            pp = nf - b * a.P;
            if (pp < 0) { --b; pp += a.P; }
            else if (pp >= a.P) { ++b; pp -= a.P; }
        };
        auto strip_setup = [&](int strip) {
            int nf, j, b, p;
            decode(strip, nf, j, b, p);
            int f0 = p - a.pad;
            f0 = f0 < 0 ? 0 : (f0 > a.T - 1 ? a.T - 1 : f0);
            const uintptr_t fb = (uintptr_t)(a.src + (size_t)(b * a.T + f0) * (size_t)(IH * IW * 3));
            fb0_lo = __builtin_amdgcn_readfirstlane((uint32_t)fb);
            fb0_hi = __builtin_amdgcn_readfirstlane((uint32_t)(fb >> 32));
#pragma unroll
            for (int dt = 0; dt < 5; ++dt) {
                int f = p + dt - a.pad;
                f = f < 0 ? 0 : (f > a.T - 1 ? a.T - 1 : f);
                fdelta[dt] = __builtin_amdgcn_readfirstlane((uint32_t)(f - f0) * (uint32_t)(IH * IW * 3));
            }
#pragma unroll
            for (int u = 0; u < 2; ++u) {
                const int row = u ? row1 : row0, g = u ? g1 : g0;
                int px = j * 96 + 4 * g;
                px = px < IW ? px : IW - 4;
                ioff[u] = (uint32_t)((row * IW + px) * 3);
            }
        };
        auto issue = [&](int rt, C1Regs& R) {
            const uint32_t roff = (uint32_t)rt * (uint32_t)(12 * IW * 3);
            const uint32_t o0 = ioff[0] + roff, o1 = ioff[1] + roff;
#pragma unroll
            for (int dt = 0; dt < 5; ++dt) {
                const uint8_t* fbu = reinterpret_cast<const uint8_t*>(((uintptr_t)fb0_lo | ((uintptr_t)fb0_hi << 32)) + fdelta[dt]);
                asm volatile("s_nop 4\n\tglobal_load_dwordx3 %0, %1, %2" : "=v"(R.w[0][dt]) : "v"(o0), "s"(fbu) : "memory");
                asm volatile("global_load_dwordx3 %0, %1, %2" : "=v"(R.w[1][dt]) : "v"(o1), "s"(fbu) : "memory");
            }
        };
        auto wait_frames = [&](C1Regs& R, int level) {
            if (level == 2) asm volatile("s_waitcnt vmcnt(11)" ::: "memory");
            else if (level == 1) asm volatile("s_waitcnt vmcnt(10)" ::: "memory");
            else asm volatile("s_waitcnt vmcnt(0)" ::: "memory");
#pragma unroll
            for (int u = 0; u < 2; ++u)
#pragma unroll
                for (int dt = 0; dt < 5; ++dt) asm volatile("" : "+v"(R.w[u][dt]));
        };
        bool zero_image[2] = {false, false};
        int* flags = reinterpret_cast<int*>(smem + OFF_INIT);
        auto cvt_write = [&](const C1Regs& R, char* buf, int slot, bool known_zero) {
            bool any;
            if (S.use_skip) {
                any = !known_zero;
            } else {
                uint32_t nz = 0;
#pragma unroll
                for (int u = 0; u < 2; ++u)
#pragma unroll
                    for (int dt = 0; dt < 5; ++dt) nz |= R.w[u][dt][0] | R.w[u][dt][1] | R.w[u][dt][2];
                any = !a.zskip || __builtin_amdgcn_ballot_w64(nz != 0) != 0;
            }
            if (lane == 0) flags[slot * 4 + (wave - 4)] = any ? 1 : 0;
            if (!any && zero_image[slot]) return;
            zero_image[slot] = !any;
#pragma unroll
            for (int u = 0; u < 2; ++u) {
                if (u == 1 && !has1) break;
                const int row = u ? row1 : row0, g = u ? g1 : g0;
#pragma unroll
                for (int q = 0; q < 4; ++q) {
                    uint32_t d[8];
#pragma unroll
                    for (int m = 0; m < 8; ++m) {
                        const int k0 = 2 * m, k1 = 2 * m + 1;
                        const int b0 = 3 * q + k0 % 3;
                        const uint32_t lo = R.w[u][k0 / 3][b0 >> 2];
                        uint32_t hi = 1u;
                        int hb = 0;
                        if (k1 < 15) {
                            const int b1 = 3 * q + k1 % 3;
                            hi = R.w[u][k1 / 3][b1 >> 2];
                            hb = b1 & 3;
                        }
                        d[m] = __builtin_amdgcn_perm(hi, lo, 0x0c000c00u | ((4u + hb) << 16) | (uint32_t)(b0 & 3));
                    }
                    const int x = 4 * g + q;
                    char* dst = buf + row * ROW_PITCH + slot_off(x);
                    *reinterpret_cast<uint4*>(dst) = uint4{d[0], d[1], d[2], d[3]};
                    *reinterpret_cast<uint4*>(dst + 16) = uint4{d[4], d[5], d[6], d[7]};
                }
            }
        };
        const int pcg = (ltid >> 4) & 7, ppw = ltid & 15;
        f16* const dump = a.dump + ((long)blockIdx.x * 256 + ltid) * 8;
        const f16x8 cz = S.use_skip ? *reinterpret_cast<const f16x8*>(a.zconst + pcg * 8) : f16x8{0, 0, 0, 0, 0, 0, 0, 0};
        const int prow = __builtin_amdgcn_readfirstlane(ltid >> 7);
        const int ccol = ltid & 31, ccg = ltid >> 5;
        const int pthr = (prow * PW + ppw) * 64 + pcg * 8;
        auto pool = [&](int strip, int rt, int t, bool fastz, bool carry_const) {
            int nf, j;
            strip_split(strip, nf, j);
            const char* cbuf = smem + OFF_CONV + (t & 1) * CONV_BYTES;
            const char* cin = smem + OFF_CARRY + ((rt & 1) ^ 1) * CARRY_BYTES;
            char* cout = smem + OFF_CARRY + (rt & 1) * CARRY_BYTES;
            auto at = [&](const char* base, int row, int cg, int col) {
                return *reinterpret_cast<const f16x8*>(base + ((row * 8 + cg) * 32 + col) * 16);
            };
            const int c0 = 2 * ppw, c1 = c0 + 1, c2 = c0 + 2 < 32 ? c0 + 2 : 31;
            f16x8 m, cnext;
            if (fastz) {
                m = at(cbuf, 0, pcg, 0);
                cnext = at(cbuf, 0, ccg, 0);
            } else {
                const f16x8 q2 = at(cbuf, 2, ccg, ccol), q3 = at(cbuf, 3, ccg, ccol);
                cnext = max8(q2, q3);
                if (prow == 0) {
                    const f16x8 a0 = carry_const ? cz : at(cin, 0, pcg, c0), a1 = carry_const ? cz : at(cin, 0, pcg, c1),
                                a2 = carry_const ? cz : at(cin, 0, pcg, c2);
                    const f16x8 b0 = at(cbuf, 0, pcg, c0), b1 = at(cbuf, 0, pcg, c1), b2 = at(cbuf, 0, pcg, c2);
                    m = max8(max8(max8(a0, a1), max8(a2, b0)), max8(b1, b2));
                } else {
                    const f16x8 a0 = at(cbuf, 0, pcg, c0), a1 = at(cbuf, 0, pcg, c1), a2 = at(cbuf, 0, pcg, c2);
                    const f16x8 b0 = at(cbuf, 1, pcg, c0), b1 = at(cbuf, 1, pcg, c1), b2 = at(cbuf, 1, pcg, c2);
                    const f16x8 d0 = at(cbuf, 2, pcg, c0), d1 = at(cbuf, 2, pcg, c1), d2 = at(cbuf, 2, pcg, c2);
                    m = max8(max8(max8(a0, a1), max8(a2, b0)), max8(max8(b1, b2), max8(max8(d0, d1), d2)));
                }
            }
            const int ph = 2 * rt - 1 + prow;
            const int pw = 16 * j + ppw;
            {
                const long ub = ((long)nf * PH + (2 * rt - 1)) * (PW * 64) + j * (16 * 64);
                f16* dst = (ph >= 0 && pw < PW) ? a.out + ub + pthr : dump;
                __builtin_nontemporal_store(m, reinterpret_cast<f16x8*>(dst));
            }
            if (ph >= 0 && j > 0 && ppw == 0) {
                f16x8 e;
                if (fastz) e = m;
                else if (prow == 0) e = max8(carry_const ? cz : at(cin, 0, pcg, 0), at(cbuf, 0, pcg, 0));
                else e = max8(max8(at(cbuf, 0, pcg, 0), at(cbuf, 1, pcg, 0)), at(cbuf, 2, pcg, 0));
                *reinterpret_cast<f16x8*>(a.edge + (((long)nf * PH + ph) * 4 + (j - 1)) * 64 + pcg * 8) = e;
            }
            *reinterpret_cast<f16x8*>(cout + (ccg * 32 + ccol) * 16) = cnext;
        };
        auto fill_skipped = [&](int strip, unsigned skip) {
            if (!skip) return;
            const int fill_lo = a.fill_partial ? 2 * conv1_s2_of_mask(skip) : 0;
            int nf, j;
            strip_split(strip, nf, j);
            const int pw = 16 * j + ppw;
            for (unsigned m = skip; m; m &= m - 1) {
                const int rt = __builtin_ctz(m);
                const int ph = 2 * rt - 1 + prow;
                if (ph >= fill_lo && pw < PW)
                    *reinterpret_cast<f16x8*>(a.out + (((long)nf * PH + ph) * PW + pw) * 64 + pcg * 8) = cz;
                if (ph >= fill_lo && j > 0 && ppw == 0)
                    *reinterpret_cast<f16x8*>(a.edge + (((long)nf * PH + ph) * 4 + (j - 1)) * 64 + pcg * 8) = cz;
            }
        };

        int* live = reinterpret_cast<int*>(smem + OFF_LIVE);
        C1Regs RA, RB;
        struct Hist { int strip, rt; unsigned skip; bool zero; bool done; };
        auto on_strip = [&](int strip, unsigned skip) {
            strip_setup(strip);
            fill_skipped(strip, skip);
        };
        Walk qi = walk_first(S, on_strip);
        auto hist = [](const Walk& q) { return Hist{q.strip, q.rt, q.skip, q.rt >= 0 && ((q.z >> q.rt) & 1u) != 0, q.done}; };
        const Hist none = {0, 0, 0u, false, true};
        Hist hA = none, hB = none, hC = none, hD = none;
        int last_rt = 0;
        auto issue_next = [&](C1Regs& R) {
            hD = hC; hC = hB; hB = hA;
            hA = hist(qi);
            if (!qi.done) last_rt = qi.rt;
            issue(last_rt, R);
            walk_next(S, qi, on_strip);
        };
        if (ltid == 0) { live[0] = qi.done ? 0 : 1; live[1] = 0; }
        const bool any_tile = !qi.done;
        issue_next(RA);
        if (any_tile) {
            wait_frames(RA, 0);
            cvt_write(RA, smem, 0, hA.zero);
        }
        issue_next(RB);
        issue_next(RA);
        bool z1 = false, z2 = false;
        auto pool_step = [&](int tprev) {
            const bool above_skipped = hD.rt > 0 && ((hD.skip >> (hD.rt - 1)) & 1u);
            const bool above_zero = hD.rt == 0 || above_skipped || z2;
            pool(hD.strip, hD.rt, tprev, z1 && above_zero, above_skipped);
        };
        int t = 0;
        while (!hC.done) {
            __syncthreads();
            const bool zc0 = tile_is_zero(smem, t);
            if (ltid == 0) live[(t + 1) & 1] = hB.done ? 0 : 1;
            wait_frames(RB, t >= 2 ? 2 : 1);
            if (!hB.done) cvt_write(RB, smem + ((t + 1) & 1) * TILE_BYTES, (t + 1) & 1, hB.zero);
            if (t > 0) pool_step(t - 1);
            issue_next(RB);
            z2 = z1; z1 = zc0;
            ++t;
            if (hC.done) break;
            __syncthreads();
            const bool zc1 = tile_is_zero(smem, t);
            if (ltid == 0) live[(t + 1) & 1] = hB.done ? 0 : 1;
            wait_frames(RA, t >= 2 ? 2 : 1);
            if (!hB.done) cvt_write(RA, smem + ((t + 1) & 1) * TILE_BYTES, (t + 1) & 1, hB.zero);
            pool_step(t - 1);
            issue_next(RA);
            z2 = z1; z1 = zc1;
            ++t;
        }
        asm volatile("s_waitcnt vmcnt(0)" ::: "memory");
        __syncthreads();
        if (t > 0) pool_step(t - 1);
        return;
    }

    if constexpr (M16) conv1_mfma_role<Mfma16>(a.Wd, a.scale, smem, lane, wave);
    else conv1_mfma_role<Mfma32>(a.Wd, a.scale, smem, lane, wave);
}

__global__ void conv1_edge_fix_kernel(f16* __restrict__ out, const f16* __restrict__ edge, long n) {
    const long idx = blockIdx.x * (long)blockDim.x + threadIdx.x;
    if (idx >= n) return;
    const int cg = idx & 7;
    const int j = (idx >> 3) & 3;
    const long rowi = idx >> 5;
    f16* o = out + (rowi * PW + 16 * j + 15) * 64 + cg * 8;
    const f16x8 e = *reinterpret_cast<const f16x8*>(edge + (rowi * 4 + j) * 64 + cg * 8);
    *reinterpret_cast<f16x8*>(o) = max8(*reinterpret_cast<const f16x8*>(o), e);
}

__device__ __forceinline__ f16 conv1_zero_patch_value(const f16* __restrict__ Wd, float scale, int c) {
    const float hi = (float)Wd[(0 * 64 + c) * 16 + 15], lo = (float)Wd[(1 * 64 + c) * 16 + 15];
    const float acc = hi * 5.9604644775390625e-8f + lo * 5.9604644775390625e-8f;
    return (f16)fmaxf(acc * scale, 0.f);
}
__global__ void conv1_zconst_kernel(const f16* __restrict__ Wd, float scale, f16* __restrict__ zconst) {
    if (threadIdx.x < 64) zconst[threadIdx.x] = conv1_zero_patch_value(Wd, scale, threadIdx.x);
}

__device__ __forceinline__ int* zmask_hdr(f16* zconst) { return reinterpret_cast<int*>(zconst); }

__global__ __launch_bounds__(256) void conv1_zero_scan_kernel(const uint8_t* __restrict__ src, unsigned* __restrict__ zmask,
                                                              const f16* __restrict__ Wd, float scale, f16* __restrict__ zconst) {
    __shared__ int rowz[IH + 2];
    const int tid = threadIdx.x, lane = tid & 63, wave = tid >> 6;
    const uint8_t* fb = src + (size_t)blockIdx.x * (size_t)(IH * IW * 3);
    for (int r = tid; r < IH; r += 256) {
        const uint4 v = *reinterpret_cast<const uint4*>(fb + (size_t)r * (IW * 3) + ((r * 37) % 90) * 16);
        rowz[r] = (v.x | v.y | v.z | v.w) == 0 ? 1 : 0;
    }
    __syncthreads();
    for (int r = wave; r < IH; r += 4) {
        if (!rowz[r]) continue;
        const uint8_t* row = fb + (size_t)r * (IW * 3);
        typedef unsigned u32x4 __attribute__((ext_vector_type(4)));
        u32x4 v = __builtin_nontemporal_load(reinterpret_cast<const u32x4*>(row + lane * 16));
        unsigned nz = v.x | v.y | v.z | v.w;
        if (lane < 26) {
            v = __builtin_nontemporal_load(reinterpret_cast<const u32x4*>(row + 1024 + lane * 16));
            nz |= v.x | v.y | v.z | v.w;
        }
        if (__builtin_amdgcn_ballot_w64(nz != 0) != 0 && lane == 0) rowz[r] = 0;
    }
    __syncthreads();
    if (wave == 0) {
        bool z = lane < ROW_TILES;
        if (z) {
            for (int r = 12 * lane; r < 12 * lane + TROWS; ++r) z = z && (r >= IH || rowz[r]);
        }
        const unsigned long long m = __builtin_amdgcn_ballot_w64(z);
        if (lane == 0) zmask[blockIdx.x] = (unsigned)m & ((1u << ROW_TILES) - 1u);
    }
    if (blockIdx.x == 0 && tid < 64) zconst[tid] = conv1_zero_patch_value(Wd, scale, tid);
    if (blockIdx.x == 0 && tid == 64) zmask_hdr(zconst)[CONV1_ROWSKIP_WORD] = 0x7fffffff;
}

__global__ void conv1_skip_mask_kernel(const unsigned* __restrict__ fz, int nclip, int T, int pad, int P, unsigned* __restrict__ skip,
                                       int* __restrict__ s2, int* __restrict__ rowskip_min) {
    const int nf = blockIdx.x * blockDim.x + threadIdx.x;
    int rs = 0x7fffffff;
    if (nf < nclip * P) {
        const int b = nf / P, p = nf - b * P;
        unsigned z = (1u << ROW_TILES) - 1u;
        for (int dt = 0; dt < 5; ++dt) {
            int f = p + dt - pad;
            f = f < 0 ? 0 : (f > T - 1 ? T - 1 : f);
            z &= fz[b * T + f];
        }
        const unsigned sk = skip_of(z);
        skip[nf] = z;
        rs = conv1_s2_of_mask(sk);
        s2[nf] = rs;
    }
#pragma unroll
    for (int d = 32; d >= 1; d >>= 1) {
        const int o = __shfl_xor(rs, d, 64);
        rs = o < rs ? o : rs;
    }
    if ((threadIdx.x & 63) == 0 && rs != 0x7fffffff) atomicMin(rowskip_min, rs);
}

size_t conv1_zmask_elems(int nclip, int T) { return (size_t)CONV1_ZHDR_WORDS + (size_t)nclip * T + 2 * (size_t)nclip * (T + 20); }
const int* conv1_s2_counts(const unsigned* zscratch, int nclip, int T, int pad) {
    return reinterpret_cast<const int*>(zscratch + CONV1_ZHDR_WORDS + (size_t)nclip * T + (size_t)nclip * (T + 2 * pad - 4));
}

hipError_t launch_conv1_scan(const uint8_t* src, int nclip, int T, int pad, const f16* Wd, float scale, unsigned* zscratch, hipStream_t s) {
    if (nclip * T <= 0) return hipSuccess;
    const int P = T + 2 * pad - 4;
    unsigned* fz = zscratch + CONV1_ZHDR_WORDS;
    unsigned* sk = fz + (size_t)nclip * T;
    f16* zc = reinterpret_cast<f16*>(zscratch);
    hipLaunchKernelGGL(conv1_zero_scan_kernel, dim3((unsigned)(nclip * T)), dim3(256), 0, s, src, fz, Wd, scale * 16777216.0f, zc);
    hipLaunchKernelGGL(conv1_skip_mask_kernel, dim3((unsigned)((nclip * P + 255) / 256)), dim3(256), 0, s, fz, nclip, T, pad, P, sk,
                       reinterpret_cast<int*>(sk + (size_t)nclip * P), reinterpret_cast<int*>(zscratch) + CONV1_ROWSKIP_WORD);
    return hipGetLastError();
}

hipError_t launch_conv1_zconst(const f16* Wd, float scale, f16* zconst, hipStream_t s) {
    hipLaunchKernelGGL(conv1_zconst_kernel, dim3(1), dim3(64), 0, s, Wd, scale * 16777216.0f, zconst);
    return hipGetLastError();
}

hipError_t launch_conv1_direct(const uint8_t* src, int nclip, int T, int pad, const f16* Wd, float scale,
                               f16* out_pooled, f16* edge, const unsigned* zscratch, bool fill_all, const EngineOpts& o, hipStream_t s) {
    static bool attr_set[64] = {};
    if (o.device < 0 || o.device >= 64) return hipErrorInvalidDevice;
    const int num_cu = o.num_cu;
    if (!attr_set[o.device]) {
        const void* ks[2] = {reinterpret_cast<const void*>(conv1_direct_kernel<false>), reinterpret_cast<const void*>(conv1_direct_kernel<true>)};
        for (const void* kf : ks) {
            hipError_t e = hipFuncSetAttribute(kf, hipFuncAttributeMaxDynamicSharedMemorySize, LDS_BYTES);
            if (e != hipSuccess) return e;
        }
        attr_set[o.device] = true;
    }
    Conv1Args a;
    a.src = src; a.nclip = nclip; a.T = T; a.pad = pad; a.P = T + 2 * pad - 4;
    a.dump = edge + (size_t)nclip * (T + 2 * pad - 4) * PH * 4 * 64;
    a.Wd = Wd; a.scale = scale * 16777216.0f; a.out = out_pooled; a.edge = edge;
    if ((long)nclip * a.P >= (1L << 24)) return hipErrorInvalidValue;
    a.nstrips = nclip * a.P * COL_TILES;
    a.invP = 1.0f / (float)a.P;
    a.zskip = o.conv1_zero_skip ? 1 : 0;
    a.zmask = nullptr;
    a.zconst = nullptr;
    a.fill_partial = 0;
    if (num_cu > MAX_WGS) return hipErrorInvalidValue;
    if (a.zskip && zscratch && nclip * T > 0 && (a.nstrips + num_cu - 1) / num_cu + 8 <= MAX_WG_STRIPS) {
        a.zmask = zscratch + CONV1_ZHDR_WORDS + (size_t)nclip * T;
        a.zconst = reinterpret_cast<const f16*>(zscratch);
        if (!fill_all) a.fill_partial = 1;
    }
    if (a.nstrips <= 0) return hipSuccess;
    if (num_cu < 8 && a.nstrips > num_cu) return hipErrorInvalidValue;
    const unsigned grid = (unsigned)(a.nstrips < num_cu ? a.nstrips : num_cu);
    if (o.conv1_mfma16) hipLaunchKernelGGL((conv1_direct_kernel<true>), dim3(grid), dim3(512), LDS_BYTES, s, a);
    else hipLaunchKernelGGL((conv1_direct_kernel<false>), dim3(grid), dim3(512), LDS_BYTES, s, a);
    return hipGetLastError();
}

hipError_t launch_conv1_edge_fix(f16* out_pooled, const f16* edge, long positions, hipStream_t s) {
    const long n = positions * PH * 4 * 8;
    if (n <= 0) return hipSuccess;
    hipLaunchKernelGGL(conv1_edge_fix_kernel, dim3((unsigned)((n + 255) / 256)), dim3(256), 0, s, out_pooled, edge, n);
    return hipGetLastError();
}

size_t conv1_edge_elems(long positions) { return (size_t)positions * PH * 4 * 64 + (size_t)MAX_WGS * DUMP_HALVES_PER_WG; }
```

### jegal_amd/csrc/elementwise_f32.hip

```cpp
#include "common.h"

__global__ void transpose_tokens_kernel(const float* __restrict__ in, int L, int D, float* __restrict__ out) {
    __shared__ float tile[32][33];
    const long n = blockIdx.z;
    const int d0 = blockIdx.x * 32, l0 = blockIdx.y * 32;
    for (int r = threadIdx.y; r < 32; r += blockDim.y) {
        const int l = l0 + r, d = d0 + threadIdx.x;
        tile[r][threadIdx.x] = (l < L && d < D) ? in[(n * L + l) * D + d] : 0.f;
    }
    __syncthreads();
    for (int r = threadIdx.y; r < 32; r += blockDim.y) {
        const int d = d0 + r, l = l0 + threadIdx.x;
        if (d < D && l < L) out[(n * D + d) * L + l] = tile[threadIdx.x][r];
    }
}

hipError_t launch_transpose_tokens(const float* in, int N, int L, int D, float* out, hipStream_t s) {
    if (N <= 0) return hipSuccess;
    hipLaunchKernelGGL(transpose_tokens_kernel, dim3((D + 31) / 32, (L + 31) / 32, N), dim3(32, 8), 0, s, in, L, D, out);
    return hipGetLastError();
}

__global__ void l2norm_kernel(const float* in, float* out, int rows, int D) {
    const int lane = threadIdx.x & 63;
    const long row = blockIdx.x * (long)(blockDim.x >> 6) + (threadIdx.x >> 6);
    if (row >= rows) return;
    const float* x = in + row * D;
    float sq = 0.f;
    for (int c = lane * 4; c < D; c += 256) {
        const f32x4 v = *reinterpret_cast<const f32x4*>(x + c);
        sq += (v.x * v.x + v.y * v.y) + (v.z * v.z + v.w * v.w);
    }
    const float nrm = fmaxf(sqrtf(wave_sum(sq)), 1e-12f);
    for (int c = lane * 4; c < D; c += 256) {
        f32x4 v = *reinterpret_cast<const f32x4*>(x + c);
        v.x /= nrm; v.y /= nrm; v.z /= nrm; v.w /= nrm;
        *reinterpret_cast<f32x4*>(out + row * D + c) = v;
    }
}

hipError_t launch_l2norm(const float* in, float* out, int rows, int D, hipStream_t s) {
    if (rows <= 0) return hipSuccess;
    hipLaunchKernelGGL(l2norm_kernel, dim3((rows + 3) / 4), dim3(256), 0, s, in, out, rows, D);
    return hipGetLastError();
}

__global__ __launch_bounds__(256) void xlmr_embed_kernel(const int32_t* __restrict__ ids, int B, int L, int D, int pad_id, int vocab, int maxpos,
                                                         const float* __restrict__ word, const float* __restrict__ pos, const float* __restrict__ type,
                                                         float* __restrict__ out) {
    const long row = blockIdx.x * 4L + (threadIdx.x >> 6);
    const int lane = threadIdx.x & 63;
    if (row >= (long)B * L) return;
    const int b = (int)(row / L), t = (int)(row - (long)b * L);
    int cnt = 0;
    for (int j = lane; j <= t; j += 64) cnt += ids[(long)b * L + j] != pad_id ? 1 : 0;
#pragma unroll
    for (int d = 32; d >= 1; d >>= 1) cnt += __shfl_xor(cnt, d, 64);
    int id = ids[row];
    int pid = id != pad_id ? pad_id + cnt : pad_id;
    id = id < 0 ? 0 : (id >= vocab ? vocab - 1 : id);
    pid = pid >= maxpos ? maxpos - 1 : pid;
    for (int c = lane * 4; c < D; c += 256) {
        const f32x4 w = *reinterpret_cast<const f32x4*>(word + (long)id * D + c);
        const f32x4 p = *reinterpret_cast<const f32x4*>(pos + (long)pid * D + c);
        const f32x4 ty = *reinterpret_cast<const f32x4*>(type + c);
        *reinterpret_cast<f32x4*>(out + row * D + c) = (w + ty) + p;
    }
}
hipError_t launch_xlmr_embed(const int32_t* ids, int B, int L, int D, int pad_id, int vocab, int maxpos, const float* word, const float* pos,
                             const float* type, float* out, hipStream_t s) {
    if (D % 4) return hipErrorInvalidValue;
    hipLaunchKernelGGL(xlmr_embed_kernel, dim3((unsigned)(((long)B * L + 3) / 4)), dim3(256), 0, s, ids, B, L, D, pad_id, vocab, maxpos, word, pos, type, out);
    return hipGetLastError();
}
__global__ void ln_stats_kernel(const float* __restrict__ part, int rows, int P, float* __restrict__ stats) {
    const int r = blockIdx.x * blockDim.x + threadIdx.x;
    if (r >= rows) return;
    double s1 = 0.0, s2 = 0.0;
    for (int p = 0; p < P; ++p) {
        const f32x2_t v = *reinterpret_cast<const f32x2_t*>(part + 2 * ((long)r * P + p));
        s1 += (double)v.x;
        s2 += (double)v.y;
    }
    const double inv_d = 1.0 / (double)(P * 64), mean = s1 * inv_d;
    double var = s2 * inv_d - mean * mean;
    var = var > 0.0 ? var : 0.0;
    *reinterpret_cast<f32x2_t*>(stats + 2 * (long)r) = f32x2_t{(float)mean, 1.f / sqrtf((float)var + 1e-5f)};
}
hipError_t launch_ln_stats(const float* part, int rows, int P, float* stats, hipStream_t s) {
    if (rows <= 0) return hipSuccess;
    hipLaunchKernelGGL(ln_stats_kernel, dim3((unsigned)((rows + 255) / 256)), dim3(256), 0, s, part, rows, P, stats);
    return hipGetLastError();
}
__global__ void mask_i32_f32_kernel(const int32_t* __restrict__ in, float* __restrict__ out, long n) {
    const long i = blockIdx.x * (long)blockDim.x + threadIdx.x;
    if (i < n) out[i] = in[i] != 0 ? 1.f : 0.f;
}
hipError_t launch_mask_i32_f32(const int32_t* in, float* out, long n, hipStream_t s) {
    hipLaunchKernelGGL(mask_i32_f32_kernel, dim3((unsigned)((n + 255) / 256)), dim3(256), 0, s, in, out, n);
    return hipGetLastError();
}

__global__ void ragged_mean_kernel(const float* __restrict__ x, const int32_t* __restrict__ off, int n, int D, float* __restrict__ out) {
    const int i = blockIdx.x;
    const int s0 = off[i], s1 = off[i + 1];
    for (int c = threadIdx.x; c < D; c += blockDim.x) {
        float acc = 0.f;
        for (int r = s0; r < s1; ++r) acc += x[(long)r * D + c];
        out[(long)i * D + c] = acc / (float)(s1 - s0);
    }
}

hipError_t launch_ragged_mean(const float* x, const int32_t* offsets, int n, int D, float* out, hipStream_t s) {
    if (n <= 0) return hipSuccess;
    hipLaunchKernelGGL(ragged_mean_kernel, dim3(n), dim3(256), 0, s, x, offsets, n, D, out);
    return hipGetLastError();
}

__global__ __launch_bounds__(256) void logmel_kernel(const float* __restrict__ wav, int n_samples, int n_frames,
                                                     const float* __restrict__ mel_basis, float* __restrict__ out) {
    __shared__ float seg[512];
    __shared__ float tc[512], ts[512];
    __shared__ float mag[257];
    const int t = blockIdx.x, b = blockIdx.y, tid = threadIdx.x;
    const float* x = wav + (long)b * n_samples;
    for (int n = tid; n < 512; n += 256) {
        float w = 0.f;
        if (n >= 96 && n < 416) w = 0.5f - 0.5f * cosf(6.283185307179586f * (float)(n - 96) / 320.f);
        int i = t * 160 + n - 256;
        if (i < 0) i = -i;
        if (i >= n_samples) i = 2 * (n_samples - 1) - i;
        i = i < 0 ? 0 : i;
        seg[n] = w * x[i];
        float sn, cs;
        sincosf(6.283185307179586f * (float)n / 512.f, &sn, &cs);
        tc[n] = cs;
        ts[n] = sn;
    }
    __syncthreads();
    for (int f = tid; f < 257; f += 256) {
        float re = 0.f, im = 0.f;
        int ph = 0;
        for (int n = 0; n < 512; ++n) {
            re += seg[n] * tc[ph];
            im -= seg[n] * ts[ph];
            ph = (ph + f) & 511;
        }
        mag[f] = sqrtf(re * re + im * im);
    }
    __syncthreads();
    if (tid < 80) {
        const float* mb = mel_basis + tid * 257;
        float acc = 0.f;
        for (int f = 0; f < 257; ++f) acc += mb[f] * mag[f];
        out[((long)b * n_frames + t) * 80 + tid] = logf(acc + 1e-20f);
    }
}

hipError_t launch_logmel(const float* wav, int B, int n_samples, const float* mel_basis, float* out, hipStream_t s) {
    const int n_frames = n_samples / 160;
    if (B <= 0 || n_frames <= 0) return hipSuccess;
    hipLaunchKernelGGL(logmel_kernel, dim3(n_frames, B), dim3(256), 0, s, wav, n_samples, n_frames, mel_basis, out);
    return hipGetLastError();
}

__global__ void mask_resize_kernel(const uint8_t* __restrict__ src, int T, int H, int W, const int* __restrict__ mask_y,
                                   uint8_t* __restrict__ dst, const long long* __restrict__ offs, long long src_bytes) {
    constexpr int OH = 270, OW = 480;
    const long idx = blockIdx.x * (long)blockDim.x + threadIdx.x;
    if (idx >= (long)T * OH * OW) return;
    const int dx = (int)(idx % OW);
    const int dy = (int)((idx / OW) % OH);
    const int f = (int)(idx / ((long)OW * OH));
    const int my = mask_y[f];
    uint8_t* o = dst + idx * 3;
    if (my < 0 && dy <= 110) {
        o[0] = o[1] = o[2] = 0;
        return;
    }
    const double scale_x = (double)W / OW, scale_y = (double)H / OH;
    float fx = (float)((dx + 0.5) * scale_x - 0.5);
    int sx = (int)floorf(fx);
    fx -= sx;
    if (sx < 0) { fx = 0.f; sx = 0; }
    if (sx + 1 >= W) { fx = 0.f; sx = W - 1; }
    float fy = (float)((dy + 0.5) * scale_y - 0.5);
    const int sy = (int)floorf(fy);
    fy -= sy;
    auto sat_short = [](float v) -> int {
        int r = __float2int_rn(v);
        return r < -32768 ? -32768 : (r > 32767 ? 32767 : r);
    };
    const int a0 = sat_short((1.f - fx) * 2048.f), a1 = sat_short(fx * 2048.f);
    const int b0 = sat_short((1.f - fy) * 2048.f), b1 = sat_short(fy * 2048.f);
    const int y0 = sy < 0 ? 0 : (sy < H ? sy : H - 1);
    const int y1 = sy + 1 < 0 ? 0 : (sy + 1 < H ? sy + 1 : H - 1);
    const int x1 = sx + 1 < W ? sx + 1 : W - 1;
    const uint8_t* fr = src + (long)f * H * W * 3;
    bool bad = false;
    if (offs) {
        const int row0 = my >= 0 ? (my + 1 < H ? my + 1 : H) : 0;
        const long long o = offs[f];
        bad = o < 0 || o + (long long)(H - row0) * W * 3 > src_bytes;
        fr = src + o - (long long)row0 * W * 3;
    }
    const bool z0 = bad || (my >= 0 && y0 <= my), z1 = bad || (my >= 0 && y1 <= my);
#pragma unroll
    for (int c = 0; c < 3; ++c) {
        const int p00 = z0 ? 0 : fr[((long)y0 * W + sx) * 3 + c], p01 = z0 ? 0 : fr[((long)y0 * W + x1) * 3 + c];
        const int p10 = z1 ? 0 : fr[((long)y1 * W + sx) * 3 + c], p11 = z1 ? 0 : fr[((long)y1 * W + x1) * 3 + c];
        const int S0 = p00 * a0 + p01 * a1, S1 = p10 * a0 + p11 * a1;
        const int v = (((b0 * (S0 >> 4)) >> 16) + ((b1 * (S1 >> 4)) >> 16) + 2) >> 2;
        o[c] = (uint8_t)(v < 0 ? 0 : (v > 255 ? 255 : v));
    }
}

constexpr int MR_RB = 6;
constexpr int MR_SPAN_MAX = 40 * 1024;
__global__ __launch_bounds__(256) void mask_resize_band_kernel(const uint8_t* __restrict__ src, int T, int H, int W, const int* __restrict__ mask_y,
                                                               uint8_t* __restrict__ dst, const long long* __restrict__ offs, long long src_bytes) {
    constexpr int OH = 270, OW = 480, RB = MR_RB;
    extern __shared__ __attribute__((aligned(16))) uint8_t mr_smem[];
    uint8_t* const orow = mr_smem;
    uint8_t* const span = mr_smem + RB * OW * 3;
    __shared__ short cx_s[OW], cx_a[OW];
    __shared__ short cx_a0[OW];
    __shared__ int ry0[RB], ry1[RB], rb0[RB], rb1[RB];
    const int tid = threadIdx.x;
    const int f = blockIdx.x / (OH / RB), band = blockIdx.x - f * (OH / RB);
    const int dy0 = band * RB;
    const int my = mask_y[f];
    uint4* out16 = reinterpret_cast<uint4*>(dst + ((long)f * OH + dy0) * (OW * 3));
    constexpr int OUT_V = RB * OW * 3 / 16;
    auto sat_short = [](float v) -> int {
        int r = __float2int_rn(v);
        return r < -32768 ? -32768 : (r > 32767 ? 32767 : r);
    };
    const double scale_x = (double)W / OW, scale_y = (double)H / OH;
    auto row_coef = [&](int dy, int& y0, int& y1, int& b0, int& b1) {
        float fy = (float)((dy + 0.5) * scale_y - 0.5);
        const int sy = (int)floorf(fy);
        fy -= sy;
        b0 = sat_short((1.f - fy) * 2048.f);
        b1 = sat_short(fy * 2048.f);
        y0 = sy < 0 ? 0 : (sy < H ? sy : H - 1);
        y1 = sy + 1 < 0 ? 0 : (sy + 1 < H ? sy + 1 : H - 1);
    };
    int ylo, yhi, t0, t1, t2;
    row_coef(dy0, ylo, t0, t1, t2);
    row_coef(dy0 + RB - 1, t0, yhi, t1, t2);
    const int row0 = my >= 0 ? (my + 1 < H ? my + 1 : H) : 0;
    const int rlo = ylo > row0 ? ylo : row0;
    const uint8_t* fr = src + (long)f * H * W * 3;
    bool bad = false;
    if (offs) {
        const long long o = offs[f];
        bad = o < 0 || o + (long long)(H - row0) * W * 3 > src_bytes;
        fr = src + o - (long long)row0 * W * 3;
    }
    const bool none = bad || rlo > yhi || (my < 0 && dy0 + RB - 1 <= 110);
    if (none) {
        for (int i = tid; i < OUT_V; i += 256) out16[i] = make_uint4(0u, 0u, 0u, 0u);
        return;
    }
    const uint8_t* p_lo = fr + (long)rlo * W * 3;
    const long nbytes = (long)(yhi - rlo + 1) * W * 3;
    const int shift = (int)((uintptr_t)p_lo & 3);
    const uint8_t* p_al = p_lo - shift;
    const long nfull = (shift + nbytes) >> 2;
    for (long i = tid; i < nfull; i += 256) reinterpret_cast<uint32_t*>(span)[i] = reinterpret_cast<const uint32_t*>(p_al)[i];
    for (long i = nfull * 4 + tid; i < shift + nbytes; i += 256) span[i] = p_al[i];
    for (int dx = tid; dx < OW; dx += 256) {
        float fx = (float)((dx + 0.5) * scale_x - 0.5);
        int sx = (int)floorf(fx);
        fx -= sx;
        if (sx < 0) { fx = 0.f; sx = 0; }
        if (sx + 1 >= W) { fx = 0.f; sx = W - 1; }
        cx_s[dx] = (short)sx;
        cx_a0[dx] = (short)sat_short((1.f - fx) * 2048.f);
        cx_a[dx] = (short)sat_short(fx * 2048.f);
    }
    if (tid < RB) row_coef(dy0 + tid, ry0[tid], ry1[tid], rb0[tid], rb1[tid]);
    __syncthreads();
    const int rowb = W * 3;
    for (int i = tid; i < RB * OW; i += 256) {
        const int r = i / OW, dx = i - r * OW;
        uint8_t* o = orow + i * 3;
        if (my < 0 && dy0 + r <= 110) {
            o[0] = o[1] = o[2] = 0;
            continue;
        }
        const int y0 = ry0[r], y1 = ry1[r], b0 = rb0[r], b1 = rb1[r];
        const int sx = cx_s[dx], a0 = cx_a0[dx], a1 = cx_a[dx];
        const int x1 = sx + 1 < W ? sx + 1 : W - 1;
        const bool z0 = my >= 0 && y0 <= my, z1 = my >= 0 && y1 <= my;
        const uint8_t* q0 = span + shift + (long)(y0 - rlo) * rowb;
        const uint8_t* q1 = span + shift + (long)(y1 - rlo) * rowb;
#pragma unroll
        for (int c = 0; c < 3; ++c) {
            const int p00 = z0 ? 0 : q0[sx * 3 + c], p01 = z0 ? 0 : q0[x1 * 3 + c];
            const int p10 = z1 ? 0 : q1[sx * 3 + c], p11 = z1 ? 0 : q1[x1 * 3 + c];
            const int S0 = p00 * a0 + p01 * a1, S1 = p10 * a0 + p11 * a1;
            const int v = (((b0 * (S0 >> 4)) >> 16) + ((b1 * (S1 >> 4)) >> 16) + 2) >> 2;
            o[c] = (uint8_t)(v < 0 ? 0 : (v > 255 ? 255 : v));
        }
    }
    __syncthreads();
    for (int i = tid; i < OUT_V; i += 256) out16[i] = reinterpret_cast<const uint4*>(orow)[i];
}

hipError_t launch_mask_resize(const uint8_t* src, int T, int H, int W, const int* mask_y_dev, uint8_t* dst, hipStream_t s,
                              const long long* offs, long long src_bytes) {
    const long n = (long)T * 270 * 480;
    if (n <= 0) return hipSuccess;
    const long span_rows = (long)(MR_RB - 1) * H / 270 + 3;
    static const bool generic = getenv("JG_MASK_RESIZE_GENERIC") != nullptr;
    if (span_rows * W * 3 + 4 <= MR_SPAN_MAX && W <= 32767 && !generic && (reinterpret_cast<uintptr_t>(src) & 3) == 0) {
        const size_t lds = (size_t)MR_RB * 480 * 3 + (((size_t)span_rows * W * 3 + 4 + 15) & ~(size_t)15);
        hipLaunchKernelGGL(mask_resize_band_kernel, dim3((unsigned)(T * (270 / MR_RB))), dim3(256), lds, s, src, T, H, W, mask_y_dev, dst, offs, src_bytes);
        return hipGetLastError();
    }
    hipLaunchKernelGGL(mask_resize_kernel, dim3((unsigned)((n + 255) / 256)), dim3(256), 0, s, src, T, H, W, mask_y_dev, dst, offs, src_bytes);
    return hipGetLastError();
}

__global__ __launch_bounds__(256) void unpack_masked_kernel(const uint8_t* __restrict__ packed, const int* __restrict__ row0,
                                                            const long long* __restrict__ offs, uint8_t* __restrict__ dst, long long packed_bytes) {
    constexpr int ROW_B = 480 * 3, ROW_V = ROW_B / 16, ROWS = 30;
    const int f = blockIdx.x;
    const int r_begin = blockIdx.y * ROWS;
    int r0 = row0[f];
    const long long of = offs[f];
    if (r0 < 0 || r0 > 270 || of < 0 || (of & 15) || (packed_bytes >= 0 && of + (long long)(270 - r0) * ROW_B > packed_bytes)) r0 = 270;
    const uint8_t* src = packed + of;
    uint8_t* out = dst + (size_t)f * (270 * ROW_B);
    typedef unsigned u32x4 __attribute__((ext_vector_type(4)));
    for (int i = threadIdx.x; i < ROWS * ROW_V; i += 256) {
        const int r = r_begin + i / ROW_V, c = i % ROW_V;
        u32x4 v = {0u, 0u, 0u, 0u};
        if (r >= r0) v = __builtin_nontemporal_load(reinterpret_cast<const u32x4*>(src + (size_t)(r - r0) * ROW_B) + c);
        reinterpret_cast<u32x4*>(out + (size_t)r * ROW_B)[c] = v;
    }
}

hipError_t launch_unpack_masked(const uint8_t* packed, const int* row0, const long long* offs, int n_frames, uint8_t* dst, hipStream_t s,
                                long long packed_bytes) {
    if (n_frames <= 0) return hipSuccess;
    hipLaunchKernelGGL(unpack_masked_kernel, dim3((unsigned)n_frames, 9), dim3(256), 0, s, packed, row0, offs, dst, packed_bytes);
    return hipGetLastError();
}

struct RowMapArgs {
    const int* s2;
    int NF, nl;
    ConvRowMap L[4];
};
__global__ __launch_bounds__(1024) void conv_rowmap_scan_kernel(RowMapArgs a) {
    __shared__ int part[4][1024];
    const int tid = threadIdx.x;
    const int per = (a.NF + 1023) / 1024;
    const int i0 = tid * per, i1 = i0 + per < a.NF ? i0 + per : a.NF;
    int sum[4] = {0, 0, 0, 0};
    for (int i = i0; i < i1; ++i) {
        const int w = a.s2[i];
#pragma unroll
        for (int l = 0; l < 4; ++l) sum[l] += (a.L[l].OH - conv_skip_decode(w, a.L[l].op)) * a.L[l].OW;
    }
#pragma unroll
    for (int l = 0; l < 4; ++l) part[l][tid] = sum[l];
    __syncthreads();
    for (int d = 1; d < 1024; d <<= 1) {
        int v[4];
#pragma unroll
        for (int l = 0; l < 4; ++l) v[l] = tid >= d ? part[l][tid - d] : 0;
        __syncthreads();
#pragma unroll
        for (int l = 0; l < 4; ++l) part[l][tid] += v[l];
        __syncthreads();
    }
    int run[4];
#pragma unroll
    for (int l = 0; l < 4; ++l) run[l] = part[l][tid] - sum[l];
    for (int i = i0; i < i1; ++i) {
        const int w = a.s2[i];
#pragma unroll
        for (int l = 0; l < 4; ++l) {
            if (l < a.nl) a.L[l].base[i] = run[l];
            run[l] += (a.L[l].OH - conv_skip_decode(w, a.L[l].op)) * a.L[l].OW;
        }
    }
    if (tid == 1023) {
#pragma unroll
        for (int l = 0; l < 4; ++l)
            if (l < a.nl) { a.L[l].base[a.NF] = part[l][1023]; *a.L[l].total = part[l][1023]; }
    }
}
__global__ __launch_bounds__(256) void conv_rowmap_fill_kernel(RowMapArgs a) {
    const int img = blockIdx.x;
    const int w = a.s2[img];
    for (int l = 0; l < a.nl; ++l) {
        const ConvRowMap& R = a.L[l];
        const int s = conv_skip_decode(w, R.op);
        const int n = (R.OH - s) * R.OW;
        const int first = img * R.OH * R.OW + s * R.OW;
        int* dst = R.map + R.base[img];
        for (int i = threadIdx.x; i < n; i += 256) dst[i] = (first + i) | (w << 24);
    }
}

hipError_t launch_conv_rowmaps(const int* s2, int NF, const ConvRowMap* layers, int nlayers, hipStream_t s) {
    if (NF <= 0 || nlayers <= 0 || nlayers > 4) return hipErrorInvalidValue;
    RowMapArgs a;
    a.s2 = s2; a.NF = NF; a.nl = nlayers;
    for (int l = 0; l < 4; ++l) {
        a.L[l] = layers[l < nlayers ? l : nlayers - 1];
        if ((long)NF * a.L[l].OH * a.L[l].OW >= (1L << 24)) return hipErrorInvalidValue;
    }
    hipLaunchKernelGGL(conv_rowmap_scan_kernel, dim3(1), dim3(1024), 0, s, a);
    hipLaunchKernelGGL(conv_rowmap_fill_kernel, dim3((unsigned)NF), dim3(256), 0, s, a);
    return hipGetLastError();
}
```

### jegal_amd/csrc/gestsync.hip

```cpp
#include "engine.h"

namespace engine {

static void gs_conv_geoms(ConvGeom g[5]) {
    g[0] = geom(FH, FW, 16, 7, 7, 3, 3, 0, 0);
    g[1] = geom(43, 78, 64, 5, 5, 2, 2, 0, 0, true);
    g[2] = geom(20, 37, 128, 3, 3, 2, 2, 1, 1, true);
    g[3] = geom(10, 19, 256, 3, 3, 1, 2, 1, 1, true);
    g[4] = geom(10, 10, 256, 3, 3, 1, 1, 1, 1, true);
}

static int gs_build_const_chain(jg_handle* h) {
    GestSyncModel& gs = h->gs;
    gs.c2C = gs.c3C = gs.c4C = gs.c5C = nullptr;
    if (!h->opts.gemm_glds || h->bf16) return JG_OK;
    constexpr int NC = 4;
    f16 *zc, *poolC, *c2C, *c3C, *c4C, *c5C;
    RET(walloc(h, gs.m, (size_t)64, &zc));
    RET(walloc(h, gs.m, (size_t)NC * 43 * 78 * 64, &poolC));
    RET(walloc(h, gs.m, (size_t)NC * 20 * 37 * 128, &c2C));
    RET(walloc(h, gs.m, (size_t)NC * 10 * 19 * 256, &c3C));
    RET(walloc(h, gs.m, (size_t)NC * 10 * 10 * 256, &c4C));
    RET(walloc(h, gs.m, (size_t)NC * 10 * 10 * 256, &c5C));
    HIPCHK(h, launch_conv1_zconst(gs.c1_direct, 1.0f / 255.0f, zc, h->stream));
    HIPCHK(h, launch_broadcast_channels(zc, 64, poolC, (long)NC * 43 * 78, h->stream));
    ConvGeom g[5];
    gs_conv_geoms(g);
    Epi e;
    e.relu = 1;
    e.out16 = c2C; RET(gemm(h, JG_ST_CONV, poolC, 0, NC * 20 * 37, gs.c2, e, &g[1]));
    e.out16 = c3C; RET(gemm(h, JG_ST_CONV, c2C, 0, NC * 10 * 19, gs.c3, e, &g[2]));
    e.out16 = c4C; RET(gemm(h, JG_ST_CONV, c3C, 0, NC * 10 * 10, gs.c4, e, &g[3]));
    e.out16 = c5C; RET(gemm(h, JG_ST_CONV, c4C, 0, NC * 10 * 10, gs.c5, e, &g[4]));
    HIPCHK(h, hipStreamSynchronize(h->stream));
    gs.c2C = c2C; gs.c3C = c3C; gs.c4C = c4C; gs.c5C = c5C;
    return JG_OK;
}

int finalize_gestsync(jg_handle* h) {
    drop_model(h, h->gs);
    GestSyncModel& gs = h->gs;
    Model& m = gs.m;
    RET(make_conv(h, m, "net_vid.conv1", "net_vid.bn1", 64, 3, 5, 7, 7, 16, 0, &gs.c1));
    RET(make_conv(h, m, "net_vid.conv2", "net_vid.bn2", 128, 64, 1, 5, 5, 64, 0, &gs.c2, 2, 2, true));
    RET(make_conv(h, m, "net_vid.conv3", "net_vid.bn3", 256, 128, 1, 3, 3, 128, 0, &gs.c3, 2, 2, true));
    RET(make_conv(h, m, "net_vid.conv4", "net_vid.bn4", 256, 256, 1, 3, 3, 256, 0, &gs.c4, 1, 2, true));
    RET(make_conv(h, m, "net_vid.conv5", "net_vid.bn5", 256, 256, 1, 3, 3, 256, 0, &gs.c5, 1, 1, true));
    RET(make_conv(h, m, "net_vid.fc6", "net_vid.bn6", 512, 256, 1, 4, 4, 256, 0, &gs.fc6));
    RET(upload(h, m, std::vector<float>(64, 1.0f / 255.0f), &gs.c1_scale255));
    if (!h->bf16) {
        std::vector<f16> hostw((size_t)64 * 784), wd((size_t)49 * 64 * 16);
        HIPCHK(h, hipMemcpy(hostw.data(), gs.c1.wh, hostw.size() * sizeof(f16), hipMemcpyDeviceToHost));
        for (int s = 0; s < 49; ++s)
            for (int o = 0; o < 64; ++o)
                for (int e = 0; e < 16; ++e) wd[((size_t)s * 64 + o) * 16 + e] = hostw[(size_t)o * 784 + s * 16 + e];
        std::vector<float> shift(64);
        HIPCHK(h, hipMemcpy(shift.data(), gs.c1.bias, 64 * sizeof(float), hipMemcpyDeviceToHost));
        for (int o = 0; o < 64; ++o) {
            const float v = shift[o] * 255.0f;
            const f16 hi = (f16)v;
            wd[((size_t)0 * 64 + o) * 16 + 15] = hi;
            wd[((size_t)1 * 64 + o) * 16 + 15] = (f16)(v - (float)hi);
        }
        RET(upload(h, m, wd, &gs.c1_direct));
    }
    RET(make_linear(h, m, "ff_vid.0.weight", "ff_vid.0.bias", 512, 512, &gs.ff0));
    RET(make_linear(h, m, "ff_vid.2.weight", "ff_vid.2.bias", 1024, 512, &gs.ff2));
    const HostTensor* pe;
    RET(need(h, "pos_encoder.pe", 50 * 512, &pe));
    RET(upload(h, m, pe->v, &gs.pe));
    for (int l = 0; l < 6; ++l) {
        const std::string p = "transformer_encoder.layers." + std::to_string(l);
        EncLayer* L = &gs.layers[l];
        RET(make_linear(h, m, p + ".self_attn.in_proj_weight", p + ".self_attn.in_proj_bias", 1536, 512, &L->qkv));
        RET(make_linear(h, m, p + ".self_attn.out_proj.weight", p + ".self_attn.out_proj.bias", 512, 512, &L->out));
        RET(make_linear(h, m, p + ".linear1.weight", p + ".linear1.bias", 2048, 512, &L->ff1));
        RET(make_linear(h, m, p + ".linear2.weight", p + ".linear2.bias", 512, 2048, &L->ff2));
        RET(make_ln(h, m, p + ".norm1.weight", p + ".norm1.bias", 512, &L->n1));
        RET(make_ln(h, m, p + ".norm2.weight", p + ".norm2.bias", 512, &L->n2));
    }
    m.ready = true;
    return gs_build_const_chain(h);
}

static int conv1_from_frames(jg_handle* h, const uint8_t* src, int nclip, int T, int pad, f16* pooled, f16* edge, unsigned* zscr, bool fill_all) {
    const bool scan = h->opts.conv1_zero_skip;
    const f16* wd = h->gs.c1_direct;
    if (debug_sync()) {
        const long NFd = (long)nclip * (T + 2 * pad - 4);
        std::fprintf(stderr, "[jg] conv1: src %p..%p pooled %p..%p edge %p..%p zscr %p..%p fill_all %d\n", (const void*)src,
                     (const void*)(src + (size_t)nclip * T * FH * FW * 3), (void*)pooled, (void*)(pooled + (size_t)NFd * 43 * 78 * 64), (void*)edge,
                     (void*)(edge + conv1_edge_elems(NFd)), (void*)zscr, (void*)(zscr + conv1_zmask_elems(nclip, T)), (int)fill_all);
    }
    if (scan) RET(timed(h, JG_ST_CONV1_AUX, [&] { return launch_conv1_scan(src, nclip, T, pad, wd, 1.0f / 255.0f, zscr, h->stream); }));
    RET(timed(h, JG_ST_CONV1, [&] { return launch_conv1_direct(src, nclip, T, pad, wd, 1.0f / 255.0f, pooled, edge,
                                                               scan ? zscr : nullptr, fill_all, h->opts, h->stream); }));
    return timed(h, JG_ST_CONV1_AUX, [&] { return launch_conv1_edge_fix(pooled, edge, (long)nclip * (T + 2 * pad - 4), h->stream); });
}

int gs_conv1_stage(jg_handle* h, const void* src, int src_u8, long sb, long st, long sh, long sw, long sc, int nclip, int T, int pad,
                   f16* pooled, bool fill_all, unsigned** zscr) {
    const long NF = (long)nclip * (T + 2 * pad - 4);
    const bool direct = src_u8 && sc == 1 && sw == 3 && sh == (long)FW * 3 && st == (long)FH * FW * 3 && sb == (long)T * st && h->conv1_direct && !h->bf16;
    *zscr = nullptr;
    if (direct) {
        f16* edge;
        RET(wsalloc(h, conv1_edge_elems(NF), &edge));
        RET(wsalloc(h, conv1_zmask_elems(nclip, T), zscr));
        return conv1_from_frames(h, static_cast<const uint8_t*>(src), nclip, T, pad, pooled, edge, *zscr, fill_all);
    }
    f16 *o1, *S;
    RET(wsalloc(h, (size_t)NF * 88 * 158 * 64, &o1));
    RET(wsalloc(h, (size_t)NF * FH * FW * 16, &S));
    ConvGeom g[5];
    gs_conv_geoms(g);
    RET(timed(h, JG_ST_STACK, [&] { return LAUNCH(h, launch_stack_frames, src, src_u8, sb, st, sh, sw, sc, nclip, T, pad, FH, FW, S, h->stream); }));
    Epi e;
    e.relu = 1; e.scale = src_u8 ? h->gs.c1_scale255 : nullptr; e.out16 = o1;
    RET(gemm(h, JG_ST_CONV1, S, 0, (int)(NF * 88 * 158), h->gs.c1, e, &g[0]));
    return timed(h, JG_ST_POOL, [&] { return LAUNCH(h, launch_maxpool3x3s2, o1, pooled, (int)NF, 88, 158, 64, h->stream, nullptr, 0, nullptr); });
}

static int gs_conv_stack(jg_handle* h, const void* src, int src_u8, long sb, long st, long sh, long sw, long sc,
                         int nclip, int T, int pad, float* conv_out, f16* conv16 = nullptr) {
    const GestSyncModel& gs = h->gs;
    const int P = T + 2 * pad - 4;
    const long NF = (long)nclip * P;
    f16 *p1, *o2, *o3, *o4, *o5, *p5;
    const int* s2pos = nullptr;
    h->last_rowskip = nullptr;
    h->last_conv_totals = nullptr;
    ConvGeom g[5];
    gs_conv_geoms(g);
    RET(wsalloc(h, (size_t)NF * 43 * 78 * 64, &p1));
    RET(wsalloc(h, (size_t)NF * 20 * 37 * 128, &o2));
    RET(wsalloc(h, (size_t)NF * 10 * 19 * 256, &o3));
    RET(wsalloc(h, (size_t)NF * 10 * 10 * 256, &o4));
    RET(wsalloc(h, (size_t)NF * 10 * 10 * 256, &o5));
    RET(wsalloc(h, (size_t)NF * 4 * 4 * 256, &p5));
    const Lin* cl[4] = {&gs.c2, &gs.c3, &gs.c4, &gs.c5};
    bool rowskip = h->opts.conv1_zero_skip && h->conv2_row_skip && gs.c2C;
    for (int l = 0; l < 4 && rowskip; ++l) {
        GemmShape q = {};
        q.set_geom(g[l + 1]);
        q.rowmap = true; q.const_in = l > 0;
        q.M = NF * g[l + 1].OH * g[l + 1].OW; q.N = cl[l]->N; q.K = q.ldw = cl[l]->K; q.ldc = cl[l]->N;
        q.w2 = run_lo(h, *cl[l], false) != nullptr; q.bias = q.out16 = true; q.relu = 1;
        rowskip = plan_gemm(q, h->opts).glds();
    }
    unsigned* zscr;
    RET(gs_conv1_stage(h, src, src_u8, sb, st, sh, sw, sc, nclip, T, pad, p1, !rowskip, &zscr));
    if (zscr && rowskip) {
        s2pos = conv1_s2_counts(zscr, nclip, T, pad);
        const f16* cin[4] = {nullptr, gs.c2C, gs.c3C, gs.c4C};
        ConvRowMap rm[4];
        int* totals;
        RET(wsalloc(h, (size_t)64, &totals));
        for (int l = 0; l < 4; ++l) {
            ConvGeom& gl = g[l + 1];
            rm[l].OH = gl.OH; rm[l].OW = gl.OW; rm[l].op = l;
            RET(wsalloc(h, (size_t)NF * gl.OH * gl.OW, &rm[l].map));
            RET(wsalloc(h, (size_t)NF + 1, &rm[l].base));
            rm[l].total = totals + l;
            gl.rowmap = rm[l].map; gl.rows_total = rm[l].total;
            gl.in_op = l - 1; gl.const_in = cin[l];
            h->last_conv_full[l] = NF * gl.OH * gl.OW;
        }
        RET(timed(h, JG_ST_CONV1_AUX, [&] { return launch_conv_rowmaps(s2pos, (int)NF, rm, 4, h->stream); }));
        h->last_conv_totals = totals;
        h->last_rowskip = reinterpret_cast<const int*>(zscr) + CONV1_ROWSKIP_WORD;
    }
    Epi e;
    e.relu = 1;
    e.out16 = o2; RET(gemm(h, JG_ST_CONV, p1, 0, (int)(NF * 20 * 37), gs.c2, e, &g[1]));
    e.out16 = o3; RET(gemm(h, JG_ST_CONV, o2, 0, (int)(NF * 10 * 19), gs.c3, e, &g[2]));
    e.out16 = o4; RET(gemm(h, JG_ST_CONV, o3, 0, (int)(NF * 10 * 10), gs.c4, e, &g[3]));
    e.out16 = o5; RET(gemm(h, JG_ST_CONV, o4, 0, (int)(NF * 10 * 10), gs.c5, e, &g[4]));
    RET(timed(h, JG_ST_POOL, [&] { return LAUNCH(h, launch_maxpool3x3s2, o5, p5, (int)NF, 10, 10, 256, h->stream, s2pos, 3, gs.c5C); }));
    e.out16 = conv16; e.out32 = conv_out;
    return gemm(h, JG_ST_CONV, p5, 4096, (int)NF, gs.fc6, e);
}

static bool gs_fused_plan(const jg_handle* h, int M, int rows_per_clip) {
    if (!h->fuse_ln || h->calib || h->bf16) return false;
    for (int l = 0; l < 6; ++l)
        if (run_lo(h, h->gs.layers[l].out, true) || run_lo(h, h->gs.layers[l].ff2, true)) return false;
    const bool clip_bias = h->precision == JG_PREC_FP16_RC;
    auto plans = [&](int N, int K, bool ln, int relu) {
        GemmShape q = {};
        q.M = M; q.N = q.ldc = N; q.K = q.lda = q.ldw = K;
        q.bias = q.out16 = true; q.relu = relu;
        q.a_tiled = !ln; q.ln_w = q.res16 = ln;
        if (clip_bias) { q.bias_clip = true; q.rpc = rows_per_clip; q.nclips = rows_per_clip > 0 ? M / rows_per_clip : 0; }
        return plan_gemm(q, h->opts).ok();
    };
    return plans(1536, 512, false, 0) && plans(512, 512, true, 0) && plans(2048, 512, false, 1) && plans(512, 2048, true, 0);
}

struct Qkv0 {
    const f16* conv16;
    int nclip, P, Twin, shift;
};

static int gs_transformer(jg_handle* h, float* x32, f16* x16, int nseq, int S, bool tiled, const Qkv0* q0 = nullptr, int rc_clips = 0,
                          const int* rc_valid = nullptr) {
    GestSyncModel& gs = h->gs;
    const int M = nseq * S;
    const int rc_rpc = rc_clips > 0 && tiled ? M / rc_clips : 0;
    if (!rc_rpc) rc_clips = 0;
    f16 *qkv, *att, *hid;
    RET(wsalloc(h, (size_t)M * 1536, &qkv));
    RET(wsalloc(h, (size_t)M * 512, &att));
    RET(wsalloc(h, (size_t)M * 2048, &hid));
    for (int l = 0; l < 6; ++l) {
        const EncLayer& L = gs.layers[l];
        if (l == 0 && q0) {
            f16* qpos;
            RET(wsalloc(h, (size_t)q0->nclip * q0->P * 1536, &qpos));
            if (!gs.qpe) RET(walloc(h, gs.m, (size_t)32 * 1536, &gs.qpe));
            f16* qpe = gs.qpe;
            Epi e;
            e.out16 = qpos; e.no_bias = 1;
            RET(gemm(h, JG_ST_GEMM, q0->conv16, 512, q0->nclip * q0->P, L.qkv, e));
            if (!gs.qpe_valid) {
                RET(timed(h, JG_ST_GEMM, [&] { return launch_pe_project(gs.pe, S, L.qkv.wh, run_lo(h, L.qkv, false), L.qkv.bias, 1536, 512, qpe, h->stream); }));
                HIPCHK(h, hipStreamSynchronize(h->stream));
                gs.qpe_valid = true;
            }
            const AttnGather ag = {qpe, q0->Twin, q0->P, q0->shift};
            RET(timed(h, JG_ST_ATTN, [&] { return launch_attention_gather(qpos, ag, nseq, S, 8, att, h->stream); }));
        } else {
            Epi e;
            e.out16 = qkv; e.a_tiled = tiled; e.rc_rpc = rc_rpc; e.rc_clips = rc_clips; e.rc_valid = rc_valid;
            RET(gemm(h, JG_ST_GEMM, x16, 512, M, L.qkv, e));
            RET(timed(h, JG_ST_ATTN, [&] { return LAUNCH(h, launch_attention, qkv, nullptr, nseq, S, 8, 64, att, h->opts, h->stream); }));
        }
        auto proj_ln = [&](const f16* A, long lda, const Lin& W, const LNp& ln) -> int {
            Epi r;
            if (tiled) {
                r.res16 = x16; r.out16 = x16; r.ln = &ln; r.ln_flavour = LN_STD;
                r.rc_rpc = rc_rpc; r.rc_clips = rc_clips; r.rc_valid = rc_valid;
                return gemm(h, JG_ST_GEMM, A, lda, M, W, r);
            }
            r.res = x32; r.ldr = 512; r.out32 = x32;
            RET(gemm(h, JG_ST_GEMM, A, lda, M, W, r));
            return timed(h, JG_ST_NORM, [&] { return LAUNCH(h, launch_layernorm, x32, ln.w, ln.b, M, 512, LN_STD, 0, x32, x16, h->stream); });
        };
        RET(proj_ln(att, 512, L.out, L.n1));
        Epi f;
        f.relu = 1; f.out16 = hid; f.a_tiled = tiled; f.rc_rpc = rc_rpc; f.rc_clips = rc_clips; f.rc_valid = rc_valid;
        RET(gemm(h, JG_ST_GEMM, x16, 512, M, L.ff1, f));
        RET(proj_ln(hid, 2048, L.ff2, L.n2));
    }
    return JG_OK;
}


static int gs_conv_stack32(jg_handle* h, const void* src, int src_u8, long sb, long st, long sh, long sw, long sc, int nclip, int T, int pad, float* conv_out) {
    const GestSyncModel& gs = h->gs;
    const int P = T + 2 * pad - 4;
    const long NF = (long)nclip * P;
    if (NF * 88 * 158 >= (1L << 31)) JG_FAIL(h, JG_ERR_ARG, "fp32 conv stack: too many positions in one pass (lower jg_set_chunk)");
    ConvGeom g[5];
    gs_conv_geoms(g);
    float *S, *o1, *p1, *o2, *o3, *o4, *o5, *p5;
    RET(wsalloc(h, (size_t)NF * FH * FW * 16, &S));
    RET(wsalloc(h, (size_t)NF * 88 * 158 * 64, &o1));
    RET(wsalloc(h, (size_t)NF * 43 * 78 * 64, &p1));
    RET(wsalloc(h, (size_t)NF * 20 * 37 * 128, &o2));
    RET(wsalloc(h, (size_t)NF * 10 * 19 * 256, &o3));
    RET(wsalloc(h, (size_t)NF * 10 * 10 * 256, &o4));
    RET(wsalloc(h, (size_t)NF * 10 * 10 * 256, &o5));
    RET(wsalloc(h, (size_t)NF * 4 * 4 * 256, &p5));
    RET(timed(h, JG_ST_STACK, [&] { return launch_stack_frames32(src, src_u8, sb, st, sh, sw, sc, nclip, T, pad, FH, FW, S, h->stream); }));
    Epi32 e;
    e.act = 1;
    RET(gemm32(h, JG_ST_CONV1, S, 0, (int)(NF * 88 * 158), gs.c1, o1, e, &g[0]));
    RET(timed(h, JG_ST_POOL, [&] { return launch_maxpool3x3s2_32(o1, p1, (int)NF, 88, 158, 64, h->stream); }));
    RET(gemm32(h, JG_ST_CONV, p1, 0, (int)(NF * 20 * 37), gs.c2, o2, e, &g[1]));
    RET(gemm32(h, JG_ST_CONV, o2, 0, (int)(NF * 10 * 19), gs.c3, o3, e, &g[2]));
    RET(gemm32(h, JG_ST_CONV, o3, 0, (int)(NF * 10 * 10), gs.c4, o4, e, &g[3]));
    RET(gemm32(h, JG_ST_CONV, o4, 0, (int)(NF * 10 * 10), gs.c5, o5, e, &g[4]));
    RET(timed(h, JG_ST_POOL, [&] { return launch_maxpool3x3s2_32(o5, p5, (int)NF, 10, 10, 256, h->stream); }));
    return gemm32(h, JG_ST_CONV, p5, 4096, (int)NF, gs.fc6, conv_out, e);
}

static int gs_transformer32(jg_handle* h, float* x32, int nseq, int S) {
    const int M = nseq * S;
    float *qkv, *att, *hid, *t;
    RET(wsalloc(h, (size_t)M * 1536, &qkv));
    RET(wsalloc(h, (size_t)M * 512, &att));
    RET(wsalloc(h, (size_t)M * 2048, &hid));
    RET(wsalloc(h, (size_t)M * 512, &t));
    for (int l = 0; l < 6; ++l) RET(post_norm_layer32(h, h->gs.layers[l], x32, t, qkv, att, hid, nullptr, nseq, S, 8, 512, 2048, 1, x32));
    return JG_OK;
}

static int gs_tail32(jg_handle* h, const float* conv, int nb, int P, int T, int shift, float** full) {
    const int S = 21, nseq = nb * T, M = nseq * S;
    float *x32, *hid;
    RET(wsalloc(h, (size_t)M * 512, &x32));
    RET(timed(h, JG_ST_MISC, [&] { return launch_window_gather(conv, h->gs.pe, nb, P, T, S, 512, shift, 0, x32, nullptr, h->stream); }));
    RET(gs_transformer32(h, x32, nseq, S));
    RET(wsalloc(h, (size_t)M * 512, &hid));
    RET(wsalloc(h, (size_t)M * 1024, full));
    Epi32 f; f.act = 1;
    RET(gemm32(h, JG_ST_GEMM, x32, 512, M, h->gs.ff0, hid, f));
    return gemm32(h, JG_ST_GEMM, hid, 512, M, h->gs.ff2, *full);
}

int gestsync_clip_impl(jg_handle* h, const void* frames, int dtype, int B, int T, float* out_feats, const int32_t* valid_host) {
    if (!h->gs.m.ready) JG_FAIL(h, JG_ERR_STATE, "GestSync weights not finalized");
    if (B <= 0 || T <= 0) JG_FAIL(h, JG_ERR_ARG, "B and T must be positive");
    if (dtype != JG_U8 && dtype != JG_F32) JG_FAIL(h, JG_ERR_ARG, "frames dtype must be JG_U8 or JG_F32");
    const int PAD = h->edge_dedup ? 4 : 12;
    const int P = T + 2 * PAD - 4, S = 21;
    const size_t esz = dtype == JG_U8 ? 1 : 4;
    const long sw = 3, sh = (long)FW * 3, st = (long)FH * FW * 3, sb = (long)T * st;
    const int am = audit_mask(h);
    const int chunk = (am & AUD_CONV) ? std::min(h->chunk, 2) : h->chunk;
    for (int b0 = 0; b0 < B; b0 += chunk) {
        const int nb = std::min(chunk, B - b0);
        h->ws.reset();
        if (h->ws_poison)
            for (auto& c : h->ws.chunks) HIPCHK(h, launch_poison(c.p, c.cap, h->stream));
        float* conv;
        RET(wsalloc(h, (size_t)nb * P * 512, &conv));
        const char* src = reinterpret_cast<const char*>(frames) + (size_t)b0 * sb * esz;
        const int nseq = nb * T, M = nseq * S;
        float* x32; f16 *x16, *hid, *mean16, *conv16 = nullptr;
        const bool tiled = !(am & AUD_GS) && gs_fused_plan(h, M, T * S);
        int* rc_valid = nullptr;
        if (valid_host && tiled && h->precision == JG_PREC_FP16_RC) {
            std::vector<int32_t> hv(nb);
            for (int b = 0; b < nb; ++b) hv[b] = valid_host[b0 + b] * S;
            RET(wsalloc(h, (size_t)nb, &rc_valid));
            RET(upload_i32_async(h, hv.data(), (size_t)nb, rc_valid));
        }
        const bool lin0 = tiled && h->qkv0_linear && h->opts.attn_mfma && T > 1;
        if (lin0) RET(wsalloc(h, (size_t)nb * P * 512, &conv16));
        if (am & AUD_CONV) {
            RET(gs_conv_stack32(h, src, dtype == JG_U8, sb, st, sh, sw, 1, nb, T, PAD, conv));
            if (conv16) RET(timed(h, JG_ST_MISC, [&] { return LAUNCH(h, launch_cast_f32_f16, (const float*)conv, conv16, (long)nb * P * 512, h->stream); }));
        } else {
            RET(gs_conv_stack(h, src, dtype == JG_U8, sb, st, sh, sw, 1, nb, T, PAD, conv, conv16));
        }
        if (am & AUD_GS) {
            float* full;
            RET(gs_tail32(h, conv, nb, P, T, 12 - PAD, &full));
            RET(timed(h, JG_ST_MISC, [&] { return launch_group_mean32(full, nseq, S, 1024, out_feats + (size_t)b0 * T * 1024, h->stream); }));
            continue;
        }
        RET(wsalloc(h, pad128(M) * 512, &x32));
        RET(wsalloc(h, pad128(M) * 512, &x16));
        RET(timed(h, JG_ST_MISC, [&] { return LAUNCH(h, launch_window_gather, conv, h->gs.pe, nb, P, T, S, 512, 12 - PAD, tiled, x32, x16, h->stream); }));
        const Qkv0 q0 = {conv16, nb, P, T, 12 - PAD};
        RET(gs_transformer(h, x32, x16, nseq, S, tiled, lin0 ? &q0 : nullptr, nb, rc_valid));
        RET(wsalloc(h, (size_t)M * 512, &hid));
        RET(wsalloc(h, (size_t)nseq * 512, &mean16));
        Epi f; f.relu = 1; f.out16 = hid; f.a_tiled = tiled;
        if (tiled) { f.rc_rpc = T * S; f.rc_clips = nb; f.rc_valid = rc_valid; }
        RET(gemm(h, JG_ST_GEMM, x16, 512, M, h->gs.ff0, f));
        RET(timed(h, JG_ST_MISC, [&] { return LAUNCH(h, launch_group_mean, hid, nseq, S, 512, mean16, h->stream); }));
        Epi o; o.out32 = out_feats + (size_t)b0 * T * 1024;
        RET(gemm(h, JG_ST_GEMM, mean16, 512, nseq, h->gs.ff2, o));
    }
    return JG_OK;
}

int gestsync_windows_impl(jg_handle* h, const float* x, int N, float* out, float* out_conv) {
    if (!h->gs.m.ready) JG_FAIL(h, JG_ERR_STATE, "GestSync weights not finalized");
    if (N <= 0) JG_FAIL(h, JG_ERR_ARG, "N must be positive");
    const int S = 21;
    const long sw = 1, sh = FW, st = (long)FH * FW, sc = 25 * st, sb = 3 * sc;
    const int am = audit_mask(h);
    const int wchunk = (am & AUD_CONV) ? 16 : std::max(1, h->chunk * 8);
    for (int n0 = 0; n0 < N; n0 += wchunk) {
        const int nb = std::min(wchunk, N - n0);
        h->ws.reset();
        float* conv;
        RET(wsalloc(h, (size_t)nb * S * 512, &conv));
        if (am & AUD_CONV) RET(gs_conv_stack32(h, x + (size_t)n0 * sb, 0, sb, st, sh, sw, sc, nb, 25, 0, conv));
        else RET(gs_conv_stack(h, x + (size_t)n0 * sb, 0, sb, st, sh, sw, sc, nb, 25, 0, conv));
        if (out_conv)
            RET(timed(h, JG_ST_MISC, [&] { return launch_transpose_tokens(conv, nb, S, 512, out_conv + (size_t)n0 * 512 * S, h->stream); }));
        const int M = nb * S;
        float* full;
        if (am & AUD_GS) {
            RET(gs_tail32(h, conv, nb, S, 1, 0, &full));
        } else {
            float* x32; f16 *x16, *hid;
            const bool tiled = gs_fused_plan(h, M, 0);
            RET(wsalloc(h, pad128(M) * 512, &x32));
            RET(wsalloc(h, pad128(M) * 512, &x16));
            RET(timed(h, JG_ST_MISC, [&] { return LAUNCH(h, launch_window_gather, conv, h->gs.pe, nb, S, 1, S, 512, 0, tiled, x32, x16, h->stream); }));
            RET(gs_transformer(h, x32, x16, nb, S, tiled));
            RET(wsalloc(h, (size_t)M * 512, &hid));
            RET(wsalloc(h, (size_t)M * 1024, &full));
            Epi f; f.relu = 1; f.out16 = hid; f.a_tiled = tiled;
            RET(gemm(h, JG_ST_GEMM, x16, 512, M, h->gs.ff0, f));
            Epi o; o.out32 = full;
            RET(gemm(h, JG_ST_GEMM, hid, 512, M, h->gs.ff2, o));
        }
        RET(timed(h, JG_ST_MISC, [&] { return launch_transpose_tokens(full, nb, S, 1024, out + (size_t)n0 * 1024 * S, h->stream); }));
    }
    return JG_OK;
}

}
```

### jegal_amd/csrc/shared.h

```cpp
#pragma once
#include <hip/hip_runtime.h>
#include <stdint.h>
#include <cstdio>

__host__ __device__ inline int conv_skip_decode(int w, int op) {
    const int s3 = w / 2;
    const int s = op == 0 ? w : s3 - (op - 1);
    return s > 0 ? s : 0;
}
struct ConvRowMap {
    int OH, OW, op;
    int* map;
    int* base;
    int* total;
};
constexpr int CONV1_ZHDR_WORDS = 64;
constexpr int CONV1_ROWSKIP_WORD = 32;

enum { LN_STD = 0, LN_ANNOTATED = 1 };

struct EngineOpts {
    int device = 0;
    int num_cu = 256;
    const void* zeros = nullptr;
    bool gemm_glds = true;
    bool gemm_persistent = true;
    bool gemm_big_tile = true, gemm_small_tile = true, gemm_tall_tile = true;
    int gemm_tile = 0;
    int gemm_counted = 1;
    int gemm_stagger = 0;
    bool lanes_active = false;
    bool attn_mfma = true;
    bool conv1_zero_skip = true;
    bool conv1_mfma16 = true;
    char* kname = nullptr;
};
constexpr int KNAME_LEN = 96;
template <class... T>
inline void record_kernel(char* kname, const char* fmt, T... v) {
    if (kname) snprintf(kname, KNAME_LEN, fmt, v...);
}
hipError_t engine_opts_init(EngineOpts& o, int device);
void engine_opts_release(EngineOpts& o);

hipError_t launch_unpack_masked(const uint8_t* packed, const int* row0, const long long* offs, int n_frames, uint8_t* dst, hipStream_t s,
                                long long packed_bytes = -1);
hipError_t launch_mask_resize(const uint8_t* src, int T, int H, int W, const int* mask_y_dev, uint8_t* dst, hipStream_t s,
                              const long long* offs = nullptr, long long src_bytes = 0);
size_t conv1_zmask_elems(int nclip, int T);
const int* conv1_s2_counts(const unsigned* zscratch, int nclip, int T, int pad);
hipError_t launch_conv_rowmaps(const int* s2, int NF, const ConvRowMap* layers, int nlayers, hipStream_t s);
size_t conv1_edge_elems(long positions);
hipError_t launch_transpose_tokens(const float* in, int N, int L, int D, float* out, hipStream_t s);
hipError_t launch_l2norm(const float* in, float* out, int rows, int D, hipStream_t s);
hipError_t launch_xlmr_embed(const int32_t* ids, int B, int L, int D, int pad_id, int vocab, int maxpos, const float* word, const float* pos,
                             const float* type, float* out, hipStream_t s);
hipError_t launch_ln_stats(const float* part, int rows, int P, float* stats, hipStream_t s);
hipError_t launch_mask_i32_f32(const int32_t* in, float* out, long n, hipStream_t s);
hipError_t launch_logmel(const float* wav, int B, int n_samples, const float* mel_basis, float* out, hipStream_t s);
size_t col_sum_scratch_elems(int K);
size_t rc_scratch_elems(int nclips, int K);
inline bool rc_bias_ok(int N, int K, int tiled) { return (K == 512 || K == 2048) && (!tiled || K == 512) && !(N & 31); }
hipError_t launch_ragged_mean(const float* x, const int32_t* offsets, int n, int D, float* out, hipStream_t s);
hipError_t launch_sim_rank(const float* e1, const float* e2, int n_local, int n_total, int row_offset, int D,
                           int32_t* rank, int32_t* ties, hipStream_t s);
hipError_t launch_spot(const float* g, const float* c, const int32_t* goff, const int32_t* coff, const int32_t* target,
                       int n, int D, float temp, int32_t* pred, float* score, hipStream_t s);
hipError_t launch_asd(const float* q, const float* cand, const int32_t* coff, int n, int D, float temp,
                      int32_t* pred2, hipStream_t s);
```

Baseline: 2534 clips/s.

## Skip conv1 leading zero rows per tile and trim unused pooled conv5 outputs

The conv1 zero mask now also records the first non-zero input row of each frame. The conv1 MFMA loop uses it to emit constant blocks for the leading all-zero part of a tile instead of computing them. The row-map scan also gains a used-extent (OHu/OWu), so the last conv layer only computes the outputs that the 3x3 stride-2 maxpool actually reads, with admitted counts kept for debugging. This adds more branching in the conv1 inner loop and changes the row-map index math, which risks correctness if the pool extents or the lead computation are off.

```diff
diff --git a/include/jegal_hip.h b/include/jegal_hip.h
--- a/include/jegal_hip.h
+++ b/include/jegal_hip.h
@@ -76,6 +76,8 @@
 int jg_debug_maxpool(jg_handle* h, const void* in, int nimg, int H, int W, int C, const int32_t* s2_host, int in_op, const void* const_in, void* out);
 int jg_debug_conv_rowmaps(jg_handle* h, const int32_t* s2_host, int NF, const int* OH, const int* OW, int nlayers, int32_t* const* map_host,
                           int32_t* const* base_host, int32_t* total_host);
+int jg_debug_conv_rowmaps_ex(jg_handle* h, const int32_t* s2_host, int NF, const int* OH, const int* OW, const int* OHu, const int* OWu, const int* op,
+                             int nlayers, int32_t* const* map_host, int32_t* const* base_host, int32_t* total_host);
 int jg_debug_gemm32(jg_handle* h, const float* A, int64_t lda, const float* W, int64_t ldw, int M, int N, int K, const float* scale,
                     const float* bias, const float* res, int64_t ldr, int res_mod, int act, float* out, int64_t ldc);
 int jg_debug_gemm_x3(jg_handle* h, const float* A, int64_t lda, const void* Wh, const void* Wl, int64_t ldw, int M, int N, int K,
@@ -86,6 +88,7 @@
 int jg_debug_last_kernel(jg_handle* h, char* buf, int len);
 int jg_debug_conv2_rowskip(jg_handle* h, int* rows);
 int jg_debug_conv_rows(jg_handle* h, int64_t* computed, int64_t* full);
+int jg_debug_conv_launch_rows(jg_handle* h, int64_t* launched, int64_t* full);
 int jg_debug_gemm(jg_handle* h, int M, int N, int K, int mode, int iters, double* ms);
 int jg_debug_gemm_ex(jg_handle* h, const void* a16, const void* w16, int M, int N, int K, int mode, int iters, double* ms);
 int jg_gestsync_windows(jg_handle* h, const float* x, int N, float* out, float* out_conv);
diff --git a/jegal_amd/_lib.py b/jegal_amd/_lib.py
--- a/jegal_amd/_lib.py
+++ b/jegal_amd/_lib.py
@@ -56,6 +56,8 @@
     "jg_debug_maxpool": [_P, _P, _I, _I, _I, _I, ctypes.POINTER(ctypes.c_int32), _I, _P, _P],
     "jg_debug_conv_rowmaps": [_P, ctypes.POINTER(ctypes.c_int32), _I, ctypes.POINTER(_I), ctypes.POINTER(_I), _I, ctypes.POINTER(_P), ctypes.POINTER(_P),
                               ctypes.POINTER(ctypes.c_int32)],
+    "jg_debug_conv_rowmaps_ex": [_P, ctypes.POINTER(ctypes.c_int32), _I, ctypes.POINTER(_I), ctypes.POINTER(_I), ctypes.POINTER(_I), ctypes.POINTER(_I),
+                                 ctypes.POINTER(_I), _I, ctypes.POINTER(_P), ctypes.POINTER(_P), ctypes.POINTER(ctypes.c_int32)],
     "jg_debug_gemm_plan": [_P, _P, _I, _I, _I, ctypes.POINTER(ctypes.c_char_p), ctypes.POINTER(_I), _I, ctypes.c_char_p, _I,
                            ctypes.POINTER(_I), ctypes.POINTER(_I), ctypes.POINTER(_I)],
     "jg_debug_weight_form": [_I, _I, _I, _I, ctypes.POINTER(_I), ctypes.POINTER(_I), ctypes.POINTER(_I)],
@@ -67,6 +69,7 @@
     "jg_debug_attention32": [_P, _P, _P, _I, _I, _I, _I, _P],
     "jg_debug_last_kernel": [_P, ctypes.c_char_p, _I],
     "jg_debug_conv_rows": [_P, ctypes.POINTER(ctypes.c_int64), ctypes.POINTER(ctypes.c_int64)],
+    "jg_debug_conv_launch_rows": [_P, ctypes.POINTER(ctypes.c_int64), ctypes.POINTER(ctypes.c_int64)],
     "jg_jegal_gestures": [_P, _P, _P, _I, _I, _I, _P],
     "jg_jegal_audio": [_P, _P, _I, _I, _P],
     "jg_jegal_audio_ragged": [_P, _P, _I, _I, ctypes.POINTER(ctypes.c_int32), _P],
@@ -357,7 +360,7 @@
             s2 = (ctypes.c_int32 * nimg)(*s2)
         self._ck(self.lib.jg_debug_maxpool(self.h, _ptr(x), nimg, H, W, C, s2, int(in_op), _ptr(const_in), _ptr(out)))
 
-    def debug_conv_rowmaps(self, s2_host, layers, fill=-1):
+    def debug_conv_rowmaps(self, s2_host, layers, fill=-1, ops=None, extents=None):
         self._bind_stream()
         s2 = np.ascontiguousarray(np.asarray(s2_host, np.int32))
         NF, nl = int(s2.size), len(layers)
@@ -369,7 +372,16 @@
         OW = (_I * max(nl, 1))(*[ow for _, ow in layers])
         mp = (_P * max(nl, 1))(*[m.ctypes.data for m in maps])
         bp = (_P * max(nl, 1))(*[b.ctypes.data for b in bases])
-        self._ck(self.lib.jg_debug_conv_rowmaps(self.h, s2.ctypes.data_as(i32p), NF, OH, OW, nl, mp, bp, totals.ctypes.data_as(i32p)))
+        if ops is None and extents is None:
+            self._ck(self.lib.jg_debug_conv_rowmaps(self.h, s2.ctypes.data_as(i32p), NF, OH, OW, nl, mp, bp, totals.ctypes.data_as(i32p)))
+        else:
+            if len(ops if ops is not None else layers) != nl or len(extents if extents is not None else layers) != nl:
+                raise ValueError("debug_conv_rowmaps: ops and extents need one entry per layer")
+            op = (_I * max(nl, 1))(*[int(v) for v in ops]) if ops is not None else None
+            OHu = (_I * max(nl, 1))(*[int(e[0]) if e else 0 for e in extents]) if extents is not None else None
+            OWu = (_I * max(nl, 1))(*[int(e[1]) if e else 0 for e in extents]) if extents is not None else None
+            self._ck(self.lib.jg_debug_conv_rowmaps_ex(self.h, s2.ctypes.data_as(i32p), NF, OH, OW, OHu, OWu, op, nl, mp, bp,
+                                                       totals.ctypes.data_as(i32p)))
         return [(maps[l], bases[l], int(totals[l])) for l in range(nl)]
 
     def debug_gemm32(self, A, lda, W, ldw, M, N, K, out, ldc, scale=None, bias=None, res=None, ldr=0, res_mod=0, act=0):
@@ -407,6 +419,11 @@
     def debug_conv_rows(self):
         c, f = (ctypes.c_int64 * 4)(), (ctypes.c_int64 * 4)()
         self._ck(self.lib.jg_debug_conv_rows(self.h, c, f))
+        return list(c), list(f)
+
+    def debug_conv_launch_rows(self):
+        c, f = (ctypes.c_int64 * 4)(), (ctypes.c_int64 * 4)()
+        self._ck(self.lib.jg_debug_conv_launch_rows(self.h, c, f))
         return list(c), list(f)
 
     def debug_conv1_pool(self, frames_u8, pad):
diff --git a/jegal_amd/csrc/checks.hip b/jegal_amd/csrc/checks.hip
--- a/jegal_amd/csrc/checks.hip
+++ b/jegal_amd/csrc/checks.hip
@@ -25,6 +25,17 @@
     a.out_lo = static_cast<f16*>(c->out_lo); a.stat_out = c->stat_out;
     return a;
 }
+
+int conv_totals(jg_handle* h, int first, int64_t* rows, int64_t* full) {
+    if (!rows || !full) JG_FAIL(h, JG_ERR_ARG, "null buffer");
+    for (int l = 0; l < 4; ++l) rows[l] = full[l] = 0;
+    if (!h->last_conv_totals) return JG_OK;
+    HIPCHK(h, hipStreamSynchronize(h->stream));
+    int t[4];
+    HIPCHK(h, hipMemcpy(t, h->last_conv_totals + first, sizeof(t), hipMemcpyDeviceToHost));
+    for (int l = 0; l < 4; ++l) { rows[l] = t[l]; full[l] = h->last_conv_full[l]; }
+    return JG_OK;
+}
 }
 
 extern "C" {
@@ -41,14 +52,12 @@
 
 int jg_debug_conv_rows(jg_handle* h, int64_t* computed, int64_t* full) {
     ENTER(h);
-    if (!computed || !full) JG_FAIL(h, JG_ERR_ARG, "null buffer");
-    for (int l = 0; l < 4; ++l) computed[l] = full[l] = 0;
-    if (!h->last_conv_totals) return JG_OK;
-    HIPCHK(h, hipStreamSynchronize(h->stream));
-    int t[4];
-    HIPCHK(h, hipMemcpy(t, h->last_conv_totals, sizeof(t), hipMemcpyDeviceToHost));
-    for (int l = 0; l < 4; ++l) { computed[l] = t[l]; full[l] = h->last_conv_full[l]; }
-    return JG_OK;
+    return conv_totals(h, 4, computed, full);
+}
+
+int jg_debug_conv_launch_rows(jg_handle* h, int64_t* launched, int64_t* full) {
+    ENTER(h);
+    return conv_totals(h, 0, launched, full);
 }
 
 int jg_debug_conv1_pool(jg_handle* h, const void* frames_u8, int B, int T, int pad, void* out_f16) {
@@ -210,14 +219,20 @@
 
 int jg_debug_conv_rowmaps(jg_handle* h, const int32_t* s2_host, int NF, const int* OH, const int* OW, int nlayers, int32_t* const* map_host,
                           int32_t* const* base_host, int32_t* total_host) {
+    return jg_debug_conv_rowmaps_ex(h, s2_host, NF, OH, OW, nullptr, nullptr, nullptr, nlayers, map_host, base_host, total_host);
+}
+
+int jg_debug_conv_rowmaps_ex(jg_handle* h, const int32_t* s2_host, int NF, const int* OH, const int* OW, const int* OHu, const int* OWu, const int* op,
+                             int nlayers, int32_t* const* map_host, int32_t* const* base_host, int32_t* total_host) {
     ENTER(h);
     h->kname[0] = 0;
     if (!s2_host || !OH || !OW || !map_host || !base_host || !total_host || NF <= 0) JG_FAIL(h, JG_ERR_ARG, "jg_debug_conv_rowmaps: bad arguments");
     if (nlayers < 1 || nlayers > 4) JG_FAIL(h, JG_ERR_ARG, "launch_conv_rowmaps: the launcher rejects this shape / argument set");
     for (int l = 0; l < nlayers; ++l) {
-        if (OH[l] <= 0 || OW[l] <= 0 || !map_host[l] || !base_host[l]) JG_FAIL(h, JG_ERR_ARG, "jg_debug_conv_rowmaps: bad layer %d", l);
+        if (OH[l] <= 0 || OW[l] <= 0 || !map_host[l] || !base_host[l] || (op && (op[l] < 0 || op[l] > 3)))
+            JG_FAIL(h, JG_ERR_ARG, "jg_debug_conv_rowmaps: bad layer %d", l);
         for (int i = 0; i < NF; ++i)
-            if (s2_host[i] < 0 || s2_host[i] > 255 || conv_skip_decode(s2_host[i], l) > OH[l])
+            if (s2_host[i] < 0 || s2_host[i] > 255 || conv_skip_decode(s2_host[i], op ? op[l] : l) > OH[l])
                 JG_FAIL(h, JG_ERR_ARG, "jg_debug_conv_rowmaps: s2[%d] = %d outside 0..255 or past layer %d's %d rows", i, s2_host[i], l, OH[l]);
     }
     h->ws.reset();
@@ -229,7 +244,8 @@
     RET(upload_i32_async(h, s2_host, (size_t)NF, s2));
     for (int l = 0; l < nlayers; ++l) {
         const size_t n = (size_t)NF * OH[l] * OW[l];
-        rm[l].OH = OH[l]; rm[l].OW = OW[l]; rm[l].op = l;
+        rm[l].OH = OH[l]; rm[l].OW = OW[l]; rm[l].op = op ? op[l] : l;
+        rm[l].OHu = OHu ? OHu[l] : 0; rm[l].OWu = OWu ? OWu[l] : 0;
         RET(wsalloc(h, n, &rm[l].map));
         RET(wsalloc(h, (size_t)NF + 1, &rm[l].base));
         rm[l].total = totals + l;
diff --git a/jegal_amd/csrc/conv1.hip b/jegal_amd/csrc/conv1.hip
--- a/jegal_amd/csrc/conv1.hip
+++ b/jegal_amd/csrc/conv1.hip
@@ -34,6 +34,8 @@
 constexpr int TILE_BYTES = TROWS * ROW_PITCH;
 __device__ __host__ constexpr int slot_off(int x) { return 32 * x + 16 * (x / 3); }
 constexpr int ROW_TILES = 22, COL_TILES = 5;
+constexpr unsigned BAND_MASK = (1u << ROW_TILES) - 1u;
+constexpr int ZROWS_SHIFT = ROW_TILES;
 constexpr int CONV_BYTES = 4 * 8 * 32 * 16;
 constexpr int CARRY_BYTES = 8 * 32 * 16;
 constexpr int OFF_CONV = 2 * TILE_BYTES;
@@ -64,7 +66,7 @@
 struct Strips {
     int s_lo, r_hi, GX;
     const unsigned* tab;
-    bool use_skip;
+    int use_skip;
     __device__ __forceinline__ bool any() const { return s_lo < r_hi && GX > 0; }
     __device__ __forceinline__ unsigned zero_bands(int k) const {
         return use_skip ? (unsigned)__builtin_amdgcn_readfirstlane((int)tab[k]) : 0u;
@@ -76,13 +78,21 @@
     const int GX = (G32 + 7 - xcd) >> 3;
     const int per = (a.nstrips + 7) >> 3;
     const int r_lo = xcd * per, r_hi = (r_lo + per < a.nstrips) ? r_lo + per : a.nstrips;
-    return Strips{r_lo + xidx, r_hi, GX, reinterpret_cast<const unsigned*>(smem + OFF_SKIP), a.zmask != nullptr};
+    return Strips{r_lo + xidx, r_hi, GX, reinterpret_cast<const unsigned*>(smem + OFF_SKIP),
+                  __builtin_amdgcn_readfirstlane(a.zmask != nullptr ? 1 : 0)};
 }
 __device__ __forceinline__ void strip_split(int strip, int& nf, int& j) {
     nf = (int)((unsigned)strip / 5u);
     j = strip - nf * 5;
 }
-__device__ __forceinline__ unsigned skip_of(unsigned z) { return z & ((z << 1) | 1u); }
+__device__ __forceinline__ unsigned skip_of(unsigned z) {
+    z &= BAND_MASK;
+    return z & ((z << 1) | 1u);
+}
+__device__ __forceinline__ int tile_lead(unsigned z, int rt) {
+    const int d = (int)(z >> ZROWS_SHIFT) - 12 * rt;
+    return d < 0 ? 0 : (d > TROWS ? TROWS : d);
+}
 struct Walk {
     int strip, rt;
     int k;
@@ -117,8 +127,8 @@
     return q;
 }
 
-__device__ __forceinline__ bool tile_live(const char* smem, int t) {
-    return __builtin_amdgcn_readfirstlane(*reinterpret_cast<const int*>(smem + OFF_LIVE + (t & 1) * 4)) != 0;
+__device__ __forceinline__ int tile_live(const char* smem, int t) {
+    return __builtin_amdgcn_readfirstlane(*reinterpret_cast<const int*>(smem + OFF_LIVE + (t & 1) * 4));
 }
 __device__ __forceinline__ bool tile_is_zero(const char* smem, int t) {
     const int4 fl = *reinterpret_cast<const int4*>(smem + OFF_INIT + (t & 1) * 16);
@@ -236,22 +246,44 @@
 #ifdef JG_CLOCK_STAMPS
     const unsigned long long ck0 = __builtin_amdgcn_s_memtime(), rt0 = __builtin_amdgcn_s_memrealtime();
 #endif
+    auto const_block = [&](int q, char* cbuf) {
+        typename Form::Acc acc;
+        Form::zero(acc);
+#pragma unroll
+        for (int st = 0; st < 2; ++st)
+#pragma unroll
+            for (int cb = 0; cb < NCB; ++cb) F.step(acc, st, cb, F.frag((q * NSTEP + st) * NCB + cb));
+        F.store(acc, cbuf, mb0 + 2 * q, scale);
+    };
     for (int t = 0;; ++t) {
         __syncthreads();
-        if (!tile_live(smem, t)) break;
+        const int live = tile_live(smem, t);
+        if (!live) break;
         F.set_tile(smem + (t & 1) * TILE_BYTES + 3 * mb0 * ROW_PITCH);
         char* cbuf = smem + OFF_CONV + (t & 1) * CONV_BYTES;
-        if (tile_is_zero(smem, t)) {
-#pragma unroll
-            for (int q = 0; q < 2; ++q) {
-                typename Form::Acc acc;
-                Form::zero(acc);
-#pragma unroll
-                for (int st = 0; st < 2; ++st)
-#pragma unroll
-                    for (int cb = 0; cb < NCB; ++cb) F.step(acc, st, cb, F.frag((q * NSTEP + st) * NCB + cb));
-                F.store(acc, cbuf, mb0 + 2 * q, scale);
-            }
+        const int lead = live >> 8;
+        if (tile_is_zero(smem, t) || lead >= 3 * (mb0 + 2) + 7) {
+            const_block(0, cbuf);
+            const_block(1, cbuf);
+            continue;
+        }
+        if (lead >= 3 * mb0 + 7) {
+            const_block(0, cbuf);
+            f16x8 fr[DEPTH];
+#pragma unroll
+            for (int i = 0; i < DEPTH; ++i) fr[(NSTEP * NCB + i) % DEPTH] = F.frag(NSTEP * NCB + i);
+            typename Form::Acc acc;
+            Form::zero(acc);
+#pragma unroll
+            for (int st = 0; st < NSTEP; ++st)
+#pragma unroll
+                for (int cb = 0; cb < NCB; ++cb) {
+                    const int gi = (NSTEP + st) * NCB + cb;
+                    F.step(acc, st, cb, fr[gi % DEPTH]);
+                    if (gi + DEPTH < NFRAG) fr[gi % DEPTH] = F.frag(gi + DEPTH);
+                    __builtin_amdgcn_sched_barrier(0);
+                }
+            F.store(acc, cbuf, mb0 + 2, scale);
             continue;
         }
         f16x8 fr[DEPTH];
@@ -470,14 +502,20 @@
 
         int* live = reinterpret_cast<int*>(smem + OFF_LIVE);
         C1Regs RA, RB;
-        struct Hist { int strip, rt; unsigned skip; bool zero; bool done; };
+        struct Hist {
+            int strip, rt;
+            unsigned z;
+            __device__ __forceinline__ bool done() const { return strip < 0; }
+            __device__ __forceinline__ bool zero() const { return rt >= 0 && ((z >> rt) & 1u) != 0; }
+        };
         auto on_strip = [&](int strip, unsigned skip) {
             strip_setup(strip);
             fill_skipped(strip, skip);
         };
         Walk qi = walk_first(S, on_strip);
-        auto hist = [](const Walk& q) { return Hist{q.strip, q.rt, q.skip, q.rt >= 0 && ((q.z >> q.rt) & 1u) != 0, q.done}; };
-        const Hist none = {0, 0, 0u, false, true};
+        auto hist = [](const Walk& q) { return Hist{q.done ? -1 : q.strip, q.rt, q.z}; };
+        const Hist none = {-1, 0, 0u};
+        auto live_word = [](const Hist& h) { return h.done() ? 0 : 1 | (tile_lead(h.z, h.rt) << 8); };
         Hist hA = none, hB = none, hC = none, hD = none;
         int last_rt = 0;
         auto issue_next = [&](C1Regs& R) {
@@ -487,38 +525,38 @@
             issue(last_rt, R);
             walk_next(S, qi, on_strip);
         };
-        if (ltid == 0) { live[0] = qi.done ? 0 : 1; live[1] = 0; }
         const bool any_tile = !qi.done;
         issue_next(RA);
+        if (ltid == 0) { live[0] = live_word(hA); live[1] = 0; }
         if (any_tile) {
             wait_frames(RA, 0);
-            cvt_write(RA, smem, 0, hA.zero);
+            cvt_write(RA, smem, 0, hA.zero());
         }
         issue_next(RB);
         issue_next(RA);
         bool z1 = false, z2 = false;
         auto pool_step = [&](int tprev) {
-            const bool above_skipped = hD.rt > 0 && ((hD.skip >> (hD.rt - 1)) & 1u);
+            const bool above_skipped = hD.rt > 0 && ((skip_of(hD.z) >> (hD.rt - 1)) & 1u);
             const bool above_zero = hD.rt == 0 || above_skipped || z2;
             pool(hD.strip, hD.rt, tprev, z1 && above_zero, above_skipped);
         };
         int t = 0;
-        while (!hC.done) {
+        while (!hC.done()) {
             __syncthreads();
             const bool zc0 = tile_is_zero(smem, t);
-            if (ltid == 0) live[(t + 1) & 1] = hB.done ? 0 : 1;
+            if (ltid == 0) live[(t + 1) & 1] = live_word(hB);
             wait_frames(RB, t >= 2 ? 2 : 1);
-            if (!hB.done) cvt_write(RB, smem + ((t + 1) & 1) * TILE_BYTES, (t + 1) & 1, hB.zero);
+            if (!hB.done()) cvt_write(RB, smem + ((t + 1) & 1) * TILE_BYTES, (t + 1) & 1, hB.zero());
             if (t > 0) pool_step(t - 1);
             issue_next(RB);
             z2 = z1; z1 = zc0;
             ++t;
-            if (hC.done) break;
+            if (hC.done()) break;
             __syncthreads();
             const bool zc1 = tile_is_zero(smem, t);
-            if (ltid == 0) live[(t + 1) & 1] = hB.done ? 0 : 1;
+            if (ltid == 0) live[(t + 1) & 1] = live_word(hB);
             wait_frames(RA, t >= 2 ? 2 : 1);
-            if (!hB.done) cvt_write(RA, smem + ((t + 1) & 1) * TILE_BYTES, (t + 1) & 1, hB.zero);
+            if (!hB.done()) cvt_write(RA, smem + ((t + 1) & 1) * TILE_BYTES, (t + 1) & 1, hB.zero());
             pool_step(t - 1);
             issue_next(RA);
             z2 = z1; z1 = zc1;
@@ -585,7 +623,13 @@
             for (int r = 12 * lane; r < 12 * lane + TROWS; ++r) z = z && (r >= IH || rowz[r]);
         }
         const unsigned long long m = __builtin_amdgcn_ballot_w64(z);
-        if (lane == 0) zmask[blockIdx.x] = (unsigned)m & ((1u << ROW_TILES) - 1u);
+        int zr = IH;
+        for (int c = (IH - 1) / 64; c >= 0; --c) {
+            const int r = 64 * c + lane;
+            const unsigned long long nzr = __builtin_amdgcn_ballot_w64(r < IH && !rowz[r]);
+            if (nzr) zr = 64 * c + (int)__builtin_ctzll(nzr);
+        }
+        if (lane == 0) zmask[blockIdx.x] = ((unsigned)m & BAND_MASK) | ((unsigned)zr << ZROWS_SHIFT);
     }
     if (blockIdx.x == 0 && tid < 64) zconst[tid] = conv1_zero_patch_value(Wd, scale, tid);
     if (blockIdx.x == 0 && tid == 64) zmask_hdr(zconst)[CONV1_ROWSKIP_WORD] = 0x7fffffff;
@@ -597,14 +641,16 @@
     int rs = 0x7fffffff;
     if (nf < nclip * P) {
         const int b = nf / P, p = nf - b * P;
-        unsigned z = (1u << ROW_TILES) - 1u;
+        unsigned z = BAND_MASK, zr = IH;
         for (int dt = 0; dt < 5; ++dt) {
             int f = p + dt - pad;
             f = f < 0 ? 0 : (f > T - 1 ? T - 1 : f);
-            z &= fz[b * T + f];
+            const unsigned w = fz[b * T + f];
+            z &= w;
+            zr = min(zr, w >> ZROWS_SHIFT);
         }
         const unsigned sk = skip_of(z);
-        skip[nf] = z;
+        skip[nf] = z | (zr << ZROWS_SHIFT);
         rs = conv1_s2_of_mask(sk);
         s2[nf] = rs;
     }
diff --git a/jegal_amd/csrc/elementwise_f32.hip b/jegal_amd/csrc/elementwise_f32.hip
--- a/jegal_amd/csrc/elementwise_f32.hip
+++ b/jegal_amd/csrc/elementwise_f32.hip
@@ -355,19 +355,32 @@
     int NF, nl;
     ConvRowMap L[4];
 };
+__device__ inline int rowmap_pixels(const ConvRowMap& R, int w) {
+    const int s = conv_skip_decode(w, R.op);
+    return s < R.OHu ? (R.OHu - s) * R.OWu : 0;
+}
 __global__ __launch_bounds__(1024) void conv_rowmap_scan_kernel(RowMapArgs a) {
     __shared__ int part[4][1024];
+    __shared__ int admitted[4];
     const int tid = threadIdx.x;
+    if (tid < 4) admitted[tid] = 0;
+    __syncthreads();
     const int per = (a.NF + 1023) / 1024;
     const int i0 = tid * per, i1 = i0 + per < a.NF ? i0 + per : a.NF;
-    int sum[4] = {0, 0, 0, 0};
+    int sum[4] = {0, 0, 0, 0}, adm[4] = {0, 0, 0, 0};
     for (int i = i0; i < i1; ++i) {
         const int w = a.s2[i];
 #pragma unroll
-        for (int l = 0; l < 4; ++l) sum[l] += (a.L[l].OH - conv_skip_decode(w, a.L[l].op)) * a.L[l].OW;
-    }
-#pragma unroll
-    for (int l = 0; l < 4; ++l) part[l][tid] = sum[l];
+        for (int l = 0; l < 4; ++l) {
+            sum[l] += rowmap_pixels(a.L[l], w);
+            adm[l] += (a.L[l].OH - conv_skip_decode(w, a.L[l].op)) * a.L[l].OW;
+        }
+    }
+#pragma unroll
+    for (int l = 0; l < 4; ++l) {
+        part[l][tid] = sum[l];
+        if (a.L[l].admitted && adm[l]) atomicAdd(&admitted[l], adm[l]);
+    }
     __syncthreads();
     for (int d = 1; d < 1024; d <<= 1) {
         int v[4];
@@ -386,13 +399,16 @@
 #pragma unroll
         for (int l = 0; l < 4; ++l) {
             if (l < a.nl) a.L[l].base[i] = run[l];
-            run[l] += (a.L[l].OH - conv_skip_decode(w, a.L[l].op)) * a.L[l].OW;
+            run[l] += rowmap_pixels(a.L[l], w);
         }
     }
     if (tid == 1023) {
 #pragma unroll
         for (int l = 0; l < 4; ++l)
-            if (l < a.nl) { a.L[l].base[a.NF] = part[l][1023]; *a.L[l].total = part[l][1023]; }
+            if (l < a.nl) {
+                a.L[l].base[a.NF] = part[l][1023]; *a.L[l].total = part[l][1023];
+                if (a.L[l].admitted) *a.L[l].admitted = admitted[l];
+            }
     }
 }
 __global__ __launch_bounds__(256) void conv_rowmap_fill_kernel(RowMapArgs a) {
@@ -401,10 +417,10 @@
     for (int l = 0; l < a.nl; ++l) {
         const ConvRowMap& R = a.L[l];
         const int s = conv_skip_decode(w, R.op);
-        const int n = (R.OH - s) * R.OW;
+        const int n = rowmap_pixels(R, w);
         const int first = img * R.OH * R.OW + s * R.OW;
         int* dst = R.map + R.base[img];
-        for (int i = threadIdx.x; i < n; i += 256) dst[i] = (first + i) | (w << 24);
+        for (int i = threadIdx.x; i < n; i += 256) dst[i] = (first + i / R.OWu * R.OW + i % R.OWu) | (w << 24);
     }
 }
 
@@ -413,7 +429,10 @@
     RowMapArgs a;
     a.s2 = s2; a.NF = NF; a.nl = nlayers;
     for (int l = 0; l < 4; ++l) {
-        a.L[l] = layers[l < nlayers ? l : nlayers - 1];
+        ConvRowMap& R = a.L[l] = layers[l < nlayers ? l : nlayers - 1];
+        if (!R.OHu) R.OHu = R.OH;
+        if (!R.OWu) R.OWu = R.OW;
+        if (R.OHu < 1 || R.OHu > R.OH || R.OWu < 1 || R.OWu > R.OW) return hipErrorInvalidValue;
         if ((long)NF * a.L[l].OH * a.L[l].OW >= (1L << 24)) return hipErrorInvalidValue;
     }
     hipLaunchKernelGGL(conv_rowmap_scan_kernel, dim3(1), dim3(1024), 0, s, a);
diff --git a/jegal_amd/csrc/gestsync.hip b/jegal_amd/csrc/gestsync.hip
--- a/jegal_amd/csrc/gestsync.hip
+++ b/jegal_amd/csrc/gestsync.hip
@@ -159,9 +159,10 @@
         for (int l = 0; l < 4; ++l) {
             ConvGeom& gl = g[l + 1];
             rm[l].OH = gl.OH; rm[l].OW = gl.OW; rm[l].op = l;
+            if (l == 3) { rm[l].OHu = maxpool3x3s2_used(gl.OH); rm[l].OWu = maxpool3x3s2_used(gl.OW); }
             RET(wsalloc(h, (size_t)NF * gl.OH * gl.OW, &rm[l].map));
             RET(wsalloc(h, (size_t)NF + 1, &rm[l].base));
-            rm[l].total = totals + l;
+            rm[l].total = totals + l; rm[l].admitted = totals + 4 + l;
             gl.rowmap = rm[l].map; gl.rows_total = rm[l].total;
             gl.in_op = l - 1; gl.const_in = cin[l];
             h->last_conv_full[l] = NF * gl.OH * gl.OW;
@@ -176,7 +177,7 @@
     e.out16 = o3; RET(gemm(h, JG_ST_CONV, o2, 0, (int)(NF * 10 * 19), gs.c3, e, &g[2]));
     e.out16 = o4; RET(gemm(h, JG_ST_CONV, o3, 0, (int)(NF * 10 * 10), gs.c4, e, &g[3]));
     e.out16 = o5; RET(gemm(h, JG_ST_CONV, o4, 0, (int)(NF * 10 * 10), gs.c5, e, &g[4]));
-    RET(timed(h, JG_ST_POOL, [&] { return LAUNCH(h, launch_maxpool3x3s2, o5, p5, (int)NF, 10, 10, 256, h->stream, s2pos, 3, gs.c5C); }));
+    RET(timed(h, JG_ST_POOL, [&] { return LAUNCH(h, launch_maxpool3x3s2, o5, p5, (int)NF, g[4].OH, g[4].OW, 256, h->stream, s2pos, 3, gs.c5C); }));
     e.out16 = conv16; e.out32 = conv_out;
     return gemm(h, JG_ST_CONV, p5, 4096, (int)NF, gs.fc6, e);
 }
diff --git a/jegal_amd/csrc/shared.h b/jegal_amd/csrc/shared.h
--- a/jegal_amd/csrc/shared.h
+++ b/jegal_amd/csrc/shared.h
@@ -10,9 +10,11 @@
 }
 struct ConvRowMap {
     int OH, OW, op;
+    int OHu = 0, OWu = 0;
     int* map;
     int* base;
     int* total;
+    int* admitted = nullptr;
 };
 constexpr int CONV1_ZHDR_WORDS = 64;
 constexpr int CONV1_ROWSKIP_WORD = 32;
@@ -49,6 +51,7 @@
                               const long long* offs = nullptr, long long src_bytes = 0);
 size_t conv1_zmask_elems(int nclip, int T);
 const int* conv1_s2_counts(const unsigned* zscratch, int nclip, int T, int pad);
+inline int maxpool3x3s2_used(int n) { return (n - 3) / 2 * 2 + 3; }
 hipError_t launch_conv_rowmaps(const int* s2, int NF, const ConvRowMap* layers, int nlayers, hipStream_t s);
 size_t conv1_edge_elems(long positions);
 hipError_t launch_transpose_tokens(const float* in, int N, int L, int D, float* out, hipStream_t s);
```

New measurement: 2546 clips/s (median of 6 runs). About the same (+0.5%).
